# OzAmram/CaloDiffusion

Hardware: AMD Instinct MI355X
Metric: sampled showers/sec (Dataset-2, 400-step DDIM) (higher is better)
Workload: dtype f32 (convs: fp32 operands as 2-term fp16 splits on the fp16 MFMA pipe, fp32 accumulate; attention/norms fp32)

## Files before the change

### calodiffusion_amd/abi.py

```python
from __future__ import annotations

import ctypes as C
import os
from typing import Optional, Sequence

import torch

_HERE = os.path.dirname(os.path.abspath(__file__))
LIB_PATH = os.environ.get("CALODIFF_LIB") or os.path.join(_HERE, "lib", "libcalodiff_hip.so")

CD_MAX_SIZES = 8
CD_ABI_VERSION = 3
TIME_KINDS = {"log": 0, "sigma": 1, "raw": 2}
OBJECTIVES = {"hybrid": 0, "noise_pred": 1, "mean_pred": 2}
LOSS_TYPES = {"l2": 0, "l1": 1, "mse": 2, "huber": 3}


class CdUnetDesc(C.Structure):
    _fields_ = [
        ("struct_size", C.c_uint32),
        ("grid", C.c_int32 * 3),
        ("in_channels", C.c_int32),
        ("n_sizes", C.c_int32),
        ("layer_sizes", C.c_int32 * CD_MAX_SIZES),
# ... 22 lines not shown

class CdLayerMlpDesc(C.Structure):
    _fields_ = [("struct_size", C.c_uint32), ("dim_in", C.c_int32), ("hidden", C.c_int32), ("cond_emb", C.c_int32), ("cond_size", C.c_int32),
                ("n_res", C.c_int32), ("time_embed_kind", C.c_int32), ("objective", C.c_int32), ("sigma_data", C.c_float)]


class CdHlfDesc(C.Structure):
    _fields_ = [("struct_size", C.c_uint32), ("n_layers", C.c_int32), ("layer_offset", C.POINTER(C.c_int32)),
                ("eta", C.POINTER(C.c_double)), ("phi", C.POINTER(C.c_double)), ("with_centres", C.POINTER(C.c_int32))]


class CdGeneratorRun(C.Structure):
    _fields_ = [("struct_size", C.c_uint32), ("batch", C.c_int32), ("energy", C.c_void_p), ("energy_is_normalised", C.c_int32),
                ("sparse_mode", C.c_int32), ("layers", C.c_void_p), ("seed", C.c_uint64), ("offset", C.c_uint64),
                ("first_row", C.c_int32), ("global_batch", C.c_int32), ("showers", C.c_void_p), ("layers_out", C.c_void_p),
                ("next_offset", C.POINTER(C.c_uint64)), ("decode_seed", C.c_uint64), ("decode_offset", C.c_uint64),
                ("next_decode_offset", C.POINTER(C.c_uint64)), ("workspace", C.c_void_p), ("workspace_bytes", C.c_size_t),
                ("stream", C.c_void_p)]


class CdClassifierDesc(C.Structure):
    _fields_ = [("struct_size", C.c_uint32), ("input_dim", C.c_int32), ("hidden", C.c_int32), ("num_layer", C.c_int32),
                ("negative_slope", C.c_float), ("dropout_p", C.c_float)]


class CdStep(C.Structure):
    _fields_ = [("sigma", C.c_float), ("sigma_prev_masked", C.c_float), ("ddim_sigma", C.c_float), ("denom", C.c_float)]


_P = C.c_void_p
_SIGNATURES = {
    "cd_last_error": (C.c_char_p, []),
    "cd_abi_version": (C.c_int, []),
    "cd_device_check": (C.c_int, [C.c_char_p, C.c_int]),
    "cd_plan_create": (C.c_int, [C.POINTER(CdUnetDesc), C.POINTER(_P)]),
    "cd_plan_destroy": (C.c_int, [_P]),
    "cd_plan_num_weights": (C.c_int, [_P, C.POINTER(C.c_int)]),
    "cd_plan_weight_name": (C.c_int, [_P, C.c_int, C.c_char_p, C.c_int, C.POINTER(C.c_int64)]),
    "cd_plan_set_weight": (C.c_int, [_P, C.c_char_p, _P, C.c_int64, _P]),
    "cd_plan_set_weights": (C.c_int, [_P, C.c_int, C.POINTER(_P), _P]),
    "cd_plan_set_coords": (C.c_int, [_P, _P, _P, _P, _P]),
    "cd_plan_workspace_bytes": (C.c_int, [_P, C.c_int, C.POINTER(C.c_size_t)]),
    "cd_unet_forward": (C.c_int, [_P, C.c_int, _P, _P, _P, _P, _P, C.c_size_t, _P]),
    "cd_denoise": (C.c_int, [_P, C.c_int, _P, _P, _P, _P, _P, C.c_size_t, _P]),
    "cd_denoise_safe": (C.c_int, [_P, C.c_int, _P, _P, _P, _P, _P, C.c_size_t, C.POINTER(C.c_int), _P]),
    "cd_ddim_sample": (C.c_int, [_P, C.c_int, _P, _P, C.POINTER(CdStep), C.c_int, _P, C.c_uint64, C.c_uint64, C.c_uint64, _P, _P, _P,
                                 C.c_int, _P, C.c_size_t, _P]),
    "cd_plan_sampler_workspace_bytes": (C.c_int, [_P, C.c_int, C.c_int, C.c_int, C.c_int, C.POINTER(C.c_size_t)]),
    "cd_sampler_run": (C.c_int, [_P, C.c_int, _P, C.c_float, _P, C.c_int, C.c_int, C.POINTER(CdSamplerOp), C.c_int,
                                 C.POINTER(C.c_int32), _P, C.c_int, _P, C.c_uint64, C.c_uint64, C.c_uint64, _P, _P, _P, C.c_int,
                                 _P, C.c_size_t, _P]),
    "cd_randn": (C.c_int, [_P, C.c_int64, C.c_uint64, C.c_uint64, _P]),
    "cd_plan_grad_layout": (C.c_int, [_P, C.c_int, C.POINTER(C.c_int64), C.POINTER(C.c_int64)]),
    "cd_plan_train_workspace_bytes": (C.c_int, [_P, C.c_int, C.POINTER(C.c_size_t)]),
    "cd_plan_status": (C.c_int, [_P, C.POINTER(C.c_int), _P]),
    "cd_layer_forward": (C.c_int, [_P, C.POINTER(C.c_void_p), C.c_int, C.c_int, _P, _P, _P, _P, _P]),
    "cd_layer_denoise": (C.c_int, [_P, C.POINTER(C.c_void_p), C.c_int, C.c_int, _P, _P, _P, _P, _P]),
    "cd_layer_sample": (C.c_int, [_P, C.POINTER(C.c_void_p), C.c_int, C.c_int, _P, _P, _P, C.c_int, _P, _P, _P, _P, _P]),
    "cd_layer_sampler_run": (C.c_int, [_P, C.POINTER(C.c_void_p), C.c_int, C.c_int, _P, C.c_float, _P, C.c_int, C.c_int, _P, C.c_int,
                                       _P, _P, C.c_int, _P, C.c_uint64, C.c_uint64, C.c_uint64, _P, _P, _P, _P]),
    "cd_layer_train_workspace_bytes": (C.c_int, [_P, C.c_int, C.POINTER(C.c_size_t)]),
    "cd_layer_train_step": (C.c_int, [_P, C.POINTER(C.c_void_p), C.c_int, C.c_int, _P, _P, _P, _P, _P, _P, _P, C.c_size_t, _P]),
    "cd_layer_train_step_loss": (C.c_int, [_P, C.POINTER(C.c_void_p), C.c_int, C.c_int, _P, _P, _P, _P, C.c_int, _P, _P, _P, C.c_size_t,
                                           _P]),
    "cd_layer_loss": (C.c_int, [_P, C.POINTER(C.c_void_p), C.c_int, C.c_int, _P, _P, _P, _P, C.c_int, _P, _P, C.c_size_t, _P]),
    "cd_layer_vjp_workspace_bytes": (C.c_int, [_P, C.c_int, C.c_int, C.POINTER(C.c_size_t)]),
    "cd_layer_denoise_vjp": (C.c_int, [_P, C.POINTER(C.c_void_p), C.c_int, C.c_int, _P, _P, _P, _P, _P, _P, _P, C.c_size_t, _P]),
    "cd_reverse_norm": (C.c_int, [_P, _P, _P, _P, C.c_int, C.POINTER(C.c_int32), C.POINTER(C.c_float), C.c_float, C.c_float, _P]),
    "cd_reverse_norm_staged": (C.c_int, [_P, _P, _P, _P, C.c_int, C.POINTER(C.c_int32), C.POINTER(C.c_float), C.c_float, C.c_float,
                                         C.c_float, C.c_float, C.c_int, _P]),
    "cd_preprocess": (C.c_int, [_P, _P, _P, _P, _P, _P, C.c_int, C.POINTER(C.c_int32), C.POINTER(C.c_float), C.c_float, C.c_float,
                                C.c_float, C.c_int, C.c_float, _P]),
    "cd_preprocess_hgcal": (C.c_int, [_P, _P, C.c_int64, _P, C.c_int, _P, _P, _P, _P, C.c_int, C.c_int, C.c_int, C.c_int,
                                      C.POINTER(C.c_double), C.c_float, C.c_float, C.c_float, C.POINTER(C.c_double),
                                      C.POINTER(C.c_double), C.c_float, _P]),
    "cd_geom_create": (C.c_int, [_P, C.c_int, C.c_int, C.c_int, C.c_int, C.POINTER(_P), _P]),
    "cd_geom_create_ex": (C.c_int, [_P, _P, C.c_int, C.c_int, C.c_int, C.c_int, C.POINTER(_P), _P]),
    "cd_geom_create_csr": (C.c_int, [_P, _P, _P, C.c_int, C.c_int, C.c_int, C.c_int, C.POINTER(_P), _P]),
    "cd_geom_refresh": (C.c_int, [_P, _P, _P]),
    "cd_geom_destroy": (C.c_int, [_P]),
    "cd_geom_apply_vjp": (C.c_int, [_P, _P, _P, _P, _P, C.c_int, C.c_float, C.c_float, C.c_int, _P]),
    "cd_geom_apply": (C.c_int, [_P, _P, _P, C.c_int, C.c_float, C.c_float, C.c_int, _P]),
    "cd_geom_sparse_workspace_bytes": (C.c_int, [_P, C.c_int, C.POINTER(C.c_size_t)]),
    "cd_geom_decode_sparse": (C.c_int, [_P, _P, _P, C.c_int, C.c_int, C.c_int, _P, C.c_uint64, C.c_uint64, _P, _P]),
    "cd_radial_create": (C.c_int, [C.c_int, _P, _P, _P, C.c_int, C.c_int, C.POINTER(_P), _P]),
    "cd_radial_destroy": (C.c_int, [_P]),
    "cd_radial_enc": (C.c_int, [_P, _P, _P, _P, C.c_int, _P]),
    "cd_radial_dec": (C.c_int, [_P, _P, _P, _P, C.c_int, _P]),
    "cd_radial_enc_vjp": (C.c_int, [_P, _P, _P, _P, _P, _P, C.c_int, _P]),
    "cd_radial_dec_vjp": (C.c_int, [_P, _P, _P, _P, _P, _P, C.c_int, _P]),
    "cd_preprocess_ds1": (C.c_int, [_P, _P, _P, _P, _P, _P, _P, _P, C.c_int, C.POINTER(C.c_double), C.c_float, C.c_float, C.c_float,
                                    C.c_int, C.c_float, _P]),
    "cd_reverse_norm_ds1": (C.c_int, [_P, _P, _P, _P, _P, _P, C.c_int, C.POINTER(C.c_double), C.c_float, C.c_float, _P]),
    "cd_plan_set_radial": (C.c_int, [_P, _P, _P, _P, C.c_int, _P]),
    "cd_plan_set_geom": (C.c_int, [_P, _P, _P, C.c_int, _P]),
    "cd_adam_step": (C.c_int, [C.c_int, C.POINTER(C.c_void_p), C.POINTER(C.c_void_p), C.POINTER(C.c_void_p), C.POINTER(C.c_void_p),
                               C.POINTER(C.c_int64), C.c_double, C.c_double, C.c_double, C.c_float, C.c_float, C.c_int, _P]),
    "cd_train_step": (C.c_int, [_P, C.c_int, _P, _P, _P, _P, C.c_int, _P, _P, _P, C.c_size_t, _P]),
    "cd_plan_vjp_workspace_bytes": (C.c_int, [_P, C.c_int, C.c_int, C.POINTER(C.c_size_t)]),
    "cd_denoise_vjp": (C.c_int, [_P, C.c_int, _P, _P, _P, _P, _P, _P, _P, C.c_size_t, _P]),
    "cd_plan_bns_workspace_bytes": (C.c_int, [_P, C.c_int, C.c_int, C.POINTER(C.c_size_t)]),
    "cd_bns_theta_grad": (C.c_int, [_P, C.c_int, C.c_int, _P, _P, _P, _P, _P, _P, _P, C.c_size_t, _P]),
    "cd_generator_create": (C.c_int, [_P, C.c_size_t, C.POINTER(_P), _P]),
    "cd_generator_destroy": (C.c_int, [_P]),
    "cd_generator_checksum": (C.c_int, [_P, C.c_size_t, C.POINTER(C.c_uint64)]),
    "cd_generator_info": (C.c_int, [_P, C.POINTER(C.c_int32)]),
    "cd_generator_geometry": (C.c_int, [_P, C.POINTER(C.c_int32)]),
    "cd_generator_workspace_bytes": (C.c_int, [_P, C.c_int, C.POINTER(C.c_size_t)]),
    "cd_generator_run": (C.c_int, [_P, C.c_int, _P, C.c_int, _P, C.c_uint64, C.c_uint64, C.c_int, C.c_int, _P, _P, C.POINTER(C.c_uint64),
                                   _P, C.c_size_t, _P]),
    "cd_generator_run_ex": (C.c_int, [_P, C.POINTER(CdGeneratorRun)]),
    "cd_hlf_create": (C.c_int, [C.POINTER(CdHlfDesc), C.POINTER(_P), _P]),
    "cd_hlf_destroy": (C.c_int, [_P]),
    "cd_hlf_compute": (C.c_int, [_P, _P, C.c_int, C.c_float, _P, _P, _P]),
    "cd_fpd_workspace_bytes": (C.c_size_t, [C.c_int, C.c_int, C.c_int]),
    "cd_fpd_moments": (C.c_int, [_P, C.c_int64, C.c_int, _P, _P, C.c_int64, C.POINTER(C.c_int32), C.c_int, _P, _P, _P, _P, C.c_size_t, _P]),
    "cd_kpd_workspace_bytes": (C.c_size_t, [C.c_int, C.c_int]),
    "cd_kpd_sums": (C.c_int, [_P, C.c_int64, C.c_int, _P, C.c_int64, C.POINTER(C.c_int32), C.c_int, C.c_double, C.c_int, _P, _P, _P, C.c_size_t,
                              _P]),
    "cd_column_histograms_workspace_bytes": (C.c_size_t, [C.c_int64, C.c_int, C.c_int]),
    "cd_column_histograms": (C.c_int, [_P, C.c_int64, C.c_int64, C.c_int, _P, C.c_int, _P, _P, C.c_size_t, _P]),
    "cd_classifier_num_params": (C.c_int, [C.POINTER(CdClassifierDesc), C.POINTER(C.c_int64)]),
    "cd_classifier_workspace_bytes": (C.c_int, [C.POINTER(CdClassifierDesc), C.c_int, C.POINTER(C.c_size_t)]),
    "cd_classifier_forward": (C.c_int, [C.POINTER(CdClassifierDesc), C.POINTER(C.c_void_p), _P, C.c_int64, _P, C.c_int64, _P, C.c_int, _P,
                                        C.c_size_t, _P]),
    "cd_classifier_train_step": (C.c_int, [C.POINTER(CdClassifierDesc), C.POINTER(C.c_void_p), _P, _P, C.c_int64, _P, C.c_int, C.c_uint64,
                                           C.c_uint64, _P, _P, C.c_int, _P, _P, C.c_double, C.c_double, C.c_double, C.c_float, C.c_int, _P,
                                           C.c_size_t, _P]),
    "cd_classifier_train_epoch": (C.c_int, [C.POINTER(CdClassifierDesc), C.POINTER(C.c_void_p), _P, _P, C.c_int64, _P, C.c_int64, C.c_int,
                                            C.c_uint64, C.c_uint64, _P, _P, _P, C.c_double, C.c_double, C.c_double, C.c_float, _P, _P,
                                            C.c_size_t, _P]),
    "cd_classifier_dropout_mask": (C.c_int, [C.c_uint64, C.c_uint64, C.c_int, C.c_float, C.c_int, C.c_int, _P, _P]),
    "cd_set_conv_precision": (C.c_int, [C.c_char_p]),
    "cd_get_conv_precision": (C.c_char_p, []),
    "cd_profile_begin": (C.c_int, []),
    "cd_profile_end": (C.c_int, [C.c_char_p, C.c_int]),
    "cd_loss_hybrid_l2": (C.c_int, [_P, C.c_int, _P, _P, _P, _P, _P, _P, C.c_size_t, _P]),
    "cd_loss_hybrid": (C.c_int, [_P, C.c_int, _P, _P, _P, _P, C.c_int, _P, _P, C.c_size_t, _P]),
    "cd_op_to_channels_last": (C.c_int, [_P, _P, C.c_int, C.c_int, C.c_int64, _P]),
    "cd_op_to_ncdhw": (C.c_int, [_P, _P, C.c_int, C.c_int, C.c_int64, _P]),
    "cd_op_cyl_conv": (C.c_int, [_P, C.c_int, _P, C.c_int, _P, _P, _P, C.c_int, C.c_int, C.POINTER(C.c_int32),
                                 C.POINTER(C.c_int32), C.POINTER(C.c_int32), _P, _P]),
    "cd_op_zslide_conv": (C.c_int, [_P, C.c_int, _P, _P, _P, _P, C.POINTER(C.c_int), C.c_int, C.c_int, C.POINTER(C.c_int32), C.c_int,
                                    _P, _P]),
    "cd_op_cyl_conv_transpose": (C.c_int, [_P, _P, _P, _P, C.c_int, C.c_int, C.POINTER(C.c_int32), C.c_int, C.c_int,
                                           C.POINTER(C.c_int32), _P, _P]),
    "cd_op_init_conv": (C.c_int, [_P, _P, _P, _P, C.c_int, C.c_int, C.c_int, C.POINTER(C.c_int32), _P, _P]),
    "cd_op_init_pair_conv": (C.c_int, [_P, _P, _P, _P, _P, C.c_int, _P, _P, _P, C.c_int, C.c_int, _P, _P, _P, C.POINTER(C.c_int), C.c_int,
                                       C.POINTER(C.c_int32), C.c_int, _P, _P]),
    "cd_op_group_norm": (C.c_int, [_P, _P, _P, _P, C.c_int, C.c_int, C.c_int64, C.c_int, C.c_int, _P, _P, _P, _P]),
    "cd_op_resnet_block": (C.c_int, [_P, C.c_int, _P, C.c_int, C.POINTER(_P), _P, _P, C.c_int, C.c_int,
                                     C.POINTER(C.c_int32), C.c_int, _P, C.c_size_t, _P]),
    "cd_op_linear_attention": (C.c_int, [_P, C.POINTER(_P), _P, C.c_int, C.c_int, C.POINTER(C.c_int32), _P, C.c_size_t, _P]),
    "cd_op_conv_backward": (C.c_int, [_P, C.c_int, _P, C.c_int, _P, _P, _P, _P, _P, C.c_int, C.c_int, C.POINTER(C.c_int32),
                                      C.POINTER(C.c_int32), C.POINTER(C.c_int32), _P, C.c_size_t, _P]),
    "cd_op_conv_transpose_backward": (C.c_int, [_P, _P, _P, _P, _P, _P, C.c_int, C.c_int, C.POINTER(C.c_int32), C.c_int, C.c_int,
                                                C.POINTER(C.c_int32), _P, C.c_size_t, _P]),
    "cd_op_group_norm_backward": (C.c_int, [_P, _P, _P, _P, _P, _P, _P, _P, C.c_int, C.c_int, C.c_int64, C.c_int, C.c_int, _P,
                                            C.c_size_t, _P]),
    "cd_op_scratch_bytes": (C.c_size_t, [C.c_int, C.c_int, C.c_int64]),
    "cd_op_linear_act": (C.c_int, [_P, _P, _P, _P, C.c_int, C.c_int, C.c_int, C.c_int, C.c_float, C.c_float, C.c_uint64, C.c_uint64, C.c_int,
                                   _P]),
    "cd_op_linear_act_backward": (C.c_int, [_P, _P, _P, _P, _P, C.c_float, C.c_int, C.c_float, _P, _P, _P, C.c_int, C.c_int, C.c_int, _P,
                                            C.c_size_t, _P]),
}
EXPORTED_SYMBOLS = tuple(_SIGNATURES)

_lib = None


def load_library() -> C.CDLL:
    global _lib
    if _lib is not None:
        return _lib
    if not os.path.exists(LIB_PATH):
        raise RuntimeError(
            f"{LIB_PATH} is missing: build it with `python -m calodiffusion_amd.build` (hipcc, --offload-arch=gfx950). "
            "calodiffusion_amd has no CPU or PyTorch fallback.")
    _check_built_from_these_sources()
    lib = C.CDLL(LIB_PATH)
    for name, (res, args) in _SIGNATURES.items():
        fn = getattr(lib, name)
        fn.restype, fn.argtypes = res, args
    if lib.cd_abi_version() != CD_ABI_VERSION:
        raise RuntimeError(f"{LIB_PATH} reports ABI version {lib.cd_abi_version()}, this binding is written against "
                           f"{CD_ABI_VERSION} (include/calodiff.h): rebuild with `python -m calodiffusion_amd.build`")
    _lib = lib
    return lib


def _check_built_from_these_sources():
    if os.environ.get("CALODIFF_LIB") or os.environ.get("CD_SKIP_SRCHASH"):
        return
    from . import build
    stamp = LIB_PATH + ".srchash"
    have = open(stamp).read().strip() if os.path.exists(stamp) else None
    want = build.source_hash()
    if have != want:
        raise RuntimeError(f"{LIB_PATH} was not built from the sources in {build.CSRC} (stamp {str(have)[:12]}, sources "
                           f"{want[:12]}): run `python -m calodiffusion_amd.build`")


def _check(code: int):
    if code != 0:
        msg = load_library().cd_last_error().decode(errors="replace")
        exc = ValueError if code == -1 else RuntimeError
        raise exc(f"calodiff[{code}]: {msg}")


def require_gpu() -> str:
    lib = load_library()
    if not torch.cuda.is_available():
        raise RuntimeError("calodiffusion_amd needs an MI355X (gfx950) GPU: torch.cuda.is_available() is False and "
                           "there is no CPU fallback")
    buf = C.create_string_buffer(256)
    _check(lib.cd_device_check(buf, 256))
    return buf.value.decode()


def _ptr(t: Optional[torch.Tensor]) -> Optional[int]:
    return None if t is None else t.data_ptr()


def _stream() -> int:
    return torch.cuda.current_stream().cuda_stream


def _dev32(t: torch.Tensor, name: str) -> torch.Tensor:
    if not isinstance(t, torch.Tensor) or not t.is_cuda:
        raise RuntimeError(f"{name} must be a CUDA(ROCm) tensor: calodiffusion_amd computes on the GPU only")
    if t.dtype != torch.float32 or not t.is_contiguous():
        t = t.to(torch.float32).contiguous()
    return t


def _i32x3(v: Sequence[int]):
    return (C.c_int32 * 3)(*[int(a) for a in v])


class WorkspaceCache:

    def __init__(self):
        self._kept = {}

    def get(self, kind, key, device, nbytes) -> torch.Tensor:
        key = tuple(key)
        kept = self._kept.get(kind)
        if kept is not None and kept[0] == key and (callable(nbytes) or kept[1].numel() >= nbytes):
            return kept[1]
        del kept
        self._kept.pop(kind, None)
        ws = torch.empty(int(nbytes() if callable(nbytes) else nbytes), dtype=torch.uint8, device=device)
        self._kept[kind] = (key, ws)
        return ws

    def drop(self, *kinds):
        for kind in kinds:
            self._kept.pop(kind, None)

    def clear(self):
        self._kept.clear()

    def __iter__(self):
        return iter([(kind,) + key for kind, (key, _) in self._kept.items()])

    def __len__(self):
        return len(self._kept)


def set_conv_precision(mode: str):
    _check(load_library().cd_set_conv_precision(mode.encode()))


def get_conv_precision() -> str:
    return load_library().cd_get_conv_precision().decode()


def profile_begin():
    _check(load_library().cd_profile_begin())


def profile_end() -> dict:
    import json
    buf = C.create_string_buffer(1 << 18)
    _check(load_library().cd_profile_end(buf, 1 << 18))
    return json.loads(buf.value.decode())


def randn(shape, device, seed: int, offset: int = 0) -> torch.Tensor:
    lib = load_library()
    require_gpu()
    out = torch.empty(tuple(shape), dtype=torch.float32, device=device)
    _check(lib.cd_randn(out.data_ptr(), out.numel(), int(seed), int(offset), _stream()))
    return out
```

### calodiffusion_amd/csrc/forward.hip

```cpp
#include "plan_internal.h"
#include "kernels_attn.h"
#include "kernels_deep.h"
#include "kernels_loss.h"

#include <cstdio>
#include <cstdlib>

namespace cd {

ResP resolve(const CdPlan* p, const ResW& w, const float* emb) {
  ResP r;
  r.cin = w.cin; r.cout = w.cout; r.has_res = w.has_res;
  r.c1w3 = p->packed3(w.c1w); r.c2w3 = p->packed3(w.c2w);
  r.c1w = p->packed(w.c1w); r.c1b = p->raw(w.c1b); r.n1g = p->raw(w.n1g); r.n1b = p->raw(w.n1b);
  r.c2w = p->packed(w.c2w); r.c2b = p->raw(w.c2b); r.n2g = p->raw(w.n2g); r.n2b = p->raw(w.n2b);
  if (w.has_res) {
    r.rw = p->packed(w.rw); r.rb = p->raw(w.rb);
    if (p->packed3(w.rw)) r.rw16 = (const char*)p->packed3(w.rw) + packed_bf16x3_bytes(w.cin, w.cout, 1);
  }
  if (w.has_mlp && emb) { r.emb = emb + w.emb_off; r.emb_ld = p->emb_ld; }
  return r;
}
AttnP resolve(const CdPlan* p, const AttnW& w) {
  AttnP a;
  a.c = w.c;
  a.ng = p->raw(w.ng); a.nb = p->raw(w.nb); a.qkv = p->packed(w.qkv); a.ow = p->raw(w.ow); a.ob = p->raw(w.ob);
  a.qkv16 = (const char*)p->packed3(w.qkv) + packed_bf16x3_bytes(w.c, 96, 1);
  a.gg = p->raw(w.gg); a.gb = p->raw(w.gb);
  a.coop_sync = p->d_attn_sync;
  return a;
}

float* stats_pass(Run& r, const float* x, int C, int64_t vox, int* units) {
  const int ns = gn_nsplit_for(vox, r.B);
  float* part = r.ws->get<float>((size_t)r.B * ns * C * 2);
  if (!r.dry()) launch_ch_stats(x, part, r.B, C, vox, ns, r.s);
  *units = ns;
  return part;
}

float* conv3_with_stats(Run& r, const float* x0, int c0, const float* x1, int c1, const float* wpk, const void* wpk3,
                        const float* bias, float* out, int cout, Dims3 dims, const float* coef_in, int* units,
                        const GnDefer* defer_in, float* coef_buf, const ConvFusion::GnOut* gn_out) {
  const int64_t vox = dims.vox();
  const int cap = (int)((vox + 31) / 32);
  float* part = r.ws->get<float>((size_t)r.B * cap * cout * 2);
  int u = 0;
  if (!r.dry()) {
    ConvGeom g{dims, dims, 3, 3, 3, 1, 1, 1};
    ConvFusion fu;
    fu.coef = coef_in; fu.act = 1; fu.ch_part = part; fu.units = &u; fu.wpk_bf16x3 = wpk3; fu.status = r.status;
    if (defer_in) { fu.defer = *defer_in; fu.coef_buf = coef_buf; fu.coef = nullptr; }
    if (gn_out) fu.gn_out = *gn_out;
    launch_conv_mfma(x0, c0, x1, c1, wpk, bias, out, r.B, cout, g, r.s, fu);
    if (gn_out && *gn_out->done) {
    } else if (u == 0) {
      u = gn_nsplit_for(vox, r.B);
      if (u > cap) u = cap;
      launch_ch_stats(out, part, r.B, cout, vox, u, r.s);
    }
  }
  *units = u;
  return part;
}

static float* conv3_x_half_with_stats(Run& r, const float* x0, int c0, int c1, const void* wpk3, float* out, int cout, Dims3 dims,
                                      int* units) {
  const int64_t vox = dims.vox();
  const int cap = (int)((vox + 31) / 32);
  float* part = r.ws->get<float>((size_t)r.B * cap * cout * 2);
  int u = 0;
  if (!r.dry()) {
    ConvGeom g{dims, dims, 3, 3, 3, 1, 1, 1};
    ConvFusion fu;
    int added = 0;
    fu.act = 1; fu.ch_part = part; fu.units = &u; fu.status = r.status; fu.add_src = out; fu.add_done = &added;
    char cat[128];
    std::snprintf(cat, sizeof cat, "conv3x3x3_s1 C%d(of %d)->%d @%dx%dx%d", c0, c0 + c1, cout, dims.d, dims.h, dims.w);
    prof::Scope scope(cat, r.s, 2.0 * 27 * c0 * cout * (double)vox * r.B, 4.0 * r.B * (double)vox * (c0 + 2 * cout));
    const bool ran = try_launch_conv_zslide(x0, c0, nullptr, 0, (const char*)wpk3 + packed_bf16x3_bytes(c0 + c1, cout, 27), nullptr, out,
                                            r.B, cout, g, r.s, fu);
    CD_REQUIRE(ran && added && u > 0, "internal: the x half of a side conv must run as a z-slide continuation");
  }
  *units = u;
  return part;
}

struct LazyClose {
  GnDefer gn;
  float* part = nullptr;
  bool on = false;
};
float* res_block(Run& r, const ResP& w, const float* x0, int c0, const float* x1, int c1, Dims3 dims,
                 float** part_out, int* units_out, LazyClose* lazy, float* h1_side, const ConvDone* h1_done) {
  Arena* ws = r.ws;
  CD_REQUIRE(c0 + c1 == w.cin, "internal: resnet block input width mismatch");
  const int64_t vox = dims.vox();
  const int G = r.groups;
  int u1 = 0, u2 = 0;
  static const bool defer_gn = getenv("CD_NO_GNDEFER") == nullptr;
  float* h1 = h1_done ? h1_done->h1 : (h1_side ? h1_side : ws->get<float>((size_t)r.B * vox * w.cout));
  const bool whole = vox <= 128 && w.cout == 32 && defer_gn && conv_precision() == PREC_F16X2 && w.c1w3 && w.c2w3;
  float* p1 = nullptr;
  CD_REQUIRE(!h1_side || (!whole && c1 > 0), "internal: a side conv belongs to a concat conv on a full-resolution grid");
  CD_REQUIRE(!h1_done || (!whole && !h1_side && c1 == 0), "internal: a finished first conv belongs to a single-input block on a full-resolution grid");
  if (h1_done) { p1 = h1_done->part; u1 = h1_done->units; }
  else if (h1_side) p1 = conv3_x_half_with_stats(r, x0, c0, c1, w.c1w3, h1, w.cout, dims, &u1);
  else if (!whole) p1 = conv3_with_stats(r, x0, c0, x1, c1, w.c1w, w.c1w3, w.c1b, h1, w.cout, dims, nullptr, &u1);
  else p1 = ws->get<float>((size_t)r.B * ((vox + 31) / 32) * w.cout * 2);
  float* coef1 = ws->get<float>((size_t)r.B * w.cout * 4);
  GnDefer d1;
  d1.part = p1; d1.units = u1; d1.gamma = w.n1g; d1.beta = w.n1b; d1.add = w.emb; d1.add_ld = w.emb_ld; d1.C = w.cout; d1.groups = G;
  d1.vox = vox;
  if (!r.dry() && !defer_gn) launch_gn_finalize(p1, u1, w.n1g, w.n1b, w.emb, w.emb_ld, coef1, r.B, w.cout, G, vox, r.s);
  float* h2 = ws->get<float>((size_t)r.B * vox * w.cout);
  const bool small = vox <= 128;
  float* po = nullptr;
  const bool no_pw_close = getenv("CD_NO_PW_CLOSE") != nullptr;
  const bool pw_close = w.has_res && !small && defer_gn && !no_pw_close && w.cout <= 128;
  const int bps = pw_close ? pointwise_units(vox) : gn_apply_blocks_per_sample(r.B, w.cout, vox);
  if (part_out) {
    po = ws->get<float>((size_t)r.B * bps * w.cout * 2);
    *part_out = po;
  }
  float* res = nullptr;
  auto shortcut_conv = [&](const GnDefer* close = nullptr) {
    if (!close) res = ws->get<float>((size_t)r.B * vox * w.cout);
    if (!r.dry()) {
      PointwiseArgs a;
      a.in0 = x0; a.ld0 = c0; a.off0 = 0; a.c0 = c0; a.in1 = x1; a.ld1 = c1; a.c1 = c1;
      a.wpk = w.rw; a.bias = w.rb; a.out = close ? h2 : res; a.batch = r.B; a.cout = w.cout; a.vox = vox;
      if (conv_precision() == PREC_F16X2 && !getenv("CD_PW_F32")) { a.wpk16 = w.rw16; a.status = r.status; }
      if (close) { a.gn_res = h2; a.gn_defer = *close; a.ch_part = po; }
      launch_pointwise(a, r.s);
    }
  };
  if (small && w.has_res) shortcut_conv();
  int fused = 0;
  if (whole && !r.dry()) {
    const float* sc0 = w.has_res ? res : x0;
    const float* sc1 = w.has_res ? nullptr : (c1 ? x1 : nullptr);
    if (try_launch_res_block_small(x0, c0, x1, c1, (const char*)w.c1w3 + packed_bf16x3_bytes(c0 + c1, 32, 27), w.c1b, w.n1g, w.n1b,
                                   w.emb, w.emb_ld, (const char*)w.c2w3 + packed_bf16x3_bytes(32, 32, 27), w.c2b, w.n2g, w.n2b, G, sc0,
                                   sc1, w.has_res ? 0 : c0, h1, h2, po, r.B, w.cout, dims, r.status, r.s))
      fused = 2;
    else
      p1 = (ws->release(p1), conv3_with_stats(r, x0, c0, x1, c1, w.c1w, w.c1w3, w.c1b, h1, w.cout, dims, nullptr, &u1));
  }
  ConvFusion::GnOut go;
  if (small && defer_gn && fused != 2) {
    go.gamma = w.n2g; go.beta = w.n2b; go.groups = G; go.part_out = po; go.done = &fused;
    if (w.has_res) { go.res0 = res; }
    else { go.res0 = x0; go.res1 = c1 ? x1 : nullptr; go.res_c0 = c0; }
  }
  float* p2 = nullptr;
  if (fused == 2) p2 = ws->get<float>((size_t)r.B * ((vox + 31) / 32) * w.cout * 2);
  else p2 = conv3_with_stats(r, h1, w.cout, nullptr, 0, w.c2w, w.c2w3, w.c2b, h2, w.cout, dims, coef1, &u2, defer_gn ? &d1 : nullptr,
                             coef1, go.gamma ? &go : nullptr);
  ws->release(p1);
  ws->release(h1);
  ws->release(coef1);
  float* coef2 = ws->get<float>((size_t)r.B * w.cout * 4);
  GnDefer d2;
  d2.part = p2; d2.units = u2; d2.gamma = w.n2g; d2.beta = w.n2b; d2.C = w.cout; d2.groups = G; d2.vox = vox;
  if (!r.dry() && !defer_gn) launch_gn_finalize(p2, u2, w.n2g, w.n2b, nullptr, 0, coef2, r.B, w.cout, G, vox, r.s);
  const GnDefer* dp2 = defer_gn ? &d2 : nullptr;
  if (part_out) *units_out = fused ? 1 : bps;
  if (pw_close) {
    shortcut_conv(&d2);
  } else if (w.has_res) {
    if (!res) shortcut_conv();
    if (!r.dry() && !fused) launch_gn_apply(h2, h2, coef2, r.B, w.cout, vox, 1, res, nullptr, 0, po, r.s, dp2);
    ws->release(res);
  } else if (lazy && !small && defer_gn && c1 == 0 && w.cout == 32 && !part_out) {
    lazy->gn = d2;
    lazy->part = p2;
    lazy->on = true;
    ws->release(coef2);
    return h2;
  } else {
    if (!r.dry() && !fused) launch_gn_apply(h2, h2, coef2, r.B, w.cout, vox, 1, x0, c1 ? x1 : nullptr, c0, po, r.s, dp2);
  }
  ws->release(p2);
  ws->release(coef2);
  return h2;
}

float* attn_block(Run& r, const AttnP& w, const float* x, Dims3 dims, float* xpart, int xunits) {
  Arena* ws = r.ws;
  const int64_t vox = dims.vox();
  const int C = w.c;
  float* own = nullptr;
  if (!xpart) {
    own = stats_pass(r, x, C, vox, &xunits);
    xpart = own;
  }
  static const bool no_fused_env = getenv("CD_NO_FUSED_ATTN") != nullptr;
  static const bool defer_env = getenv("CD_NO_GNDEFER") == nullptr;
  const bool no_fused = no_fused_env || conv_precision() != PREC_F16X2;
  const bool defer_gn = defer_env && !no_fused;
  float* coefn = ws->get<float>((size_t)r.B * C * 4);
  GnDefer dn;
  dn.part = xpart; dn.units = xunits; dn.gamma = w.ng; dn.beta = w.nb; dn.C = C; dn.groups = 1; dn.vox = vox;
  const GnDefer* dnp = defer_gn ? &dn : nullptr;
  if (!r.dry() && !defer_gn) launch_gn_finalize(xpart, xunits, w.ng, w.nb, nullptr, 0, coefn, r.B, C, 1, vox, r.s);
  const int CT = (C + 31) / 32;
  float* y = nullptr;
  float* ypart = nullptr;
  int yu = 0;
  const bool single = !no_fused && defer_gn && attn_small_eligible(vox);
  bool moments = false;
  if (!no_fused) {
    const int nsp = attn_fused_nsplit_for(vox, r.B);
    const int cap = single && nsp < 4 ? 4 : nsp;
    float* part = ws->get<float>(attn_partial_floats(r.B, cap));
    static const bool sep_combine = getenv("CD_ATTN_COMBINE_LAUNCH") != nullptr;
    const char* mom_env = getenv("CD_ATTN_MOM_MIN");
    const int64_t mom_min = mom_env ? atoll(mom_env) : (4ll << 20);
    moments = !single && !sep_combine && defer_gn && attn_moments_eligible(C) && (vox * C) % 4 == 0 && (int64_t)r.B * vox * C >= mom_min &&
              getenv("CD_NO_ATTN_MOMENTS") == nullptr;
    float* momb = moments ? ws->get<float>(attn_moment_floats(r.B, nsp)) : nullptr;
    float* wpb = ws->get<float>((size_t)r.B * CT * 1024);
    y = ws->get<float>((size_t)r.B * vox * C);
    yu = nsp;
    ypart = ws->get<float>((size_t)r.B * cap * C * 2);
    if (!r.dry() && single) {
      launch_attn_small(x, C, coefn, w.qkv16, part, w.ow, kAttnScale, w.ob, w.gg, w.gb, y, ypart, r.B, vox,
                        r.s, dnp, r.status, cap, w.coop_sync);
    } else if (!r.dry()) {
      launch_attn_kv_context(x, C, coefn, w.qkv16, part, r.B, vox, nsp, r.s, dnp, r.status, momb);
      if (sep_combine) {
        launch_attn_combine(part, nsp, w.ow, C, wpb, r.B, kAttnScale, r.s, nullptr, nullptr, true);
        launch_attn_out(x, C, coefn, w.qkv16, wpb, w.ob, y, ypart, r.B, vox, nsp, r.s, dnp, nullptr, nullptr, 0.f, r.status);
      } else {
        launch_attn_out(x, C, coefn, w.qkv16, nullptr, w.ob, y, moments ? nullptr : ypart, r.B, vox, nsp, r.s, dnp, part, w.ow,
                        kAttnScale, r.status, momb, w.gg, w.gb);
      }
    }
    if (momb) ws->release(momb);
    if (own) ws->release(own);
    own = nullptr;
    ws->release(coefn);
    ws->release(part);
    ws->release(wpb);
  } else {
    float* qkv = ws->get<float>((size_t)r.B * vox * 96);
    ws->release(coefn);
    const int nsp = attn_nsplit_for(vox, r.B);
    float* part = ws->get<float>(attn_partial_floats(r.B, nsp));
    float* wpb = ws->get<float>((size_t)r.B * CT * 1024);
    y = ws->get<float>((size_t)r.B * vox * C);
    yu = pointwise_units(vox);
    ypart = ws->get<float>((size_t)r.B * yu * C * 2);
    if (!r.dry()) launch_attn_unfused(x, C, coefn, w.qkv, w.ow, w.ob, qkv, part, nsp, wpb, y, ypart, r.B, vox, r.s);
    ws->release(part);
    ws->release(wpb);
    ws->release(qkv);
}
  if (own) ws->release(own);
  float* coefg = ws->get<float>((size_t)r.B * C * 4);
  if (!r.dry() && !single && !moments) {
    GnDefer dg;
    dg.part = ypart; dg.units = yu; dg.gamma = w.gg; dg.beta = w.gb; dg.C = C; dg.groups = 1; dg.vox = vox;
    if (!defer_gn) launch_gn_finalize(ypart, yu, w.gg, w.gb, nullptr, 0, coefg, r.B, C, 1, vox, r.s);
    launch_gn_apply(y, y, coefg, r.B, C, vox, 0, x, nullptr, 0, nullptr, r.s, defer_gn ? &dg : nullptr);
  }
  ws->release(ypart);
  ws->release(coefg);
  return y;
}

bool deep_level_desc(const CdPlan* p, const float* emb, DeepLevelDesc* out) {
  const CdUnetDesc& d = p->desc;
  const int nres = p->nres;
  if (conv_precision() != PREC_F16X2) return false;
  DeepLevelDesc L;
  L.dims = p->shapes[nres - 1];
  L.Ca = d.layer_sizes[nres - 1]; L.Cb = d.layer_sizes[nres]; L.groups = d.groups;
  const ResW* rw[6] = {&p->downs[nres - 1].r1, &p->downs[nres - 1].r2, &p->mid1, &p->mid2, &p->ups[0].r1, &p->ups[0].r2};
  for (int i = 0; i < 6; ++i) {
    const ResW& w = *rw[i];
    DeepLevelDesc::Res& r = L.res[i];
    const bool cat = i == 4;
    r.c0 = cat ? L.Cb : w.cin; r.c1 = cat ? w.cin - L.Cb : 0; r.cout = w.cout;
    if (!p->packed3(w.c1w) || !p->packed3(w.c2w)) return false;
    r.w1 = (const char*)p->packed3(w.c1w) + packed_bf16x3_bytes(w.cin, w.cout, 27);
    r.w2 = (const char*)p->packed3(w.c2w) + packed_bf16x3_bytes(w.cout, w.cout, 27);
    r.b1 = p->raw(w.c1b); r.b2 = p->raw(w.c2b); r.g1 = p->raw(w.n1g); r.be1 = p->raw(w.n1b); r.g2 = p->raw(w.n2g); r.be2 = p->raw(w.n2b);
    if (w.has_mlp && emb) { r.emb = emb + w.emb_off; r.emb_ld = p->emb_ld; }
    if (w.has_res) {
      if (!p->packed3(w.rw)) return false;
      r.wres = (const char*)p->packed3(w.rw) + packed_bf16x3_bytes(w.cin, w.cout, 1);
      r.bres = p->raw(w.rb);
    }
  }
  const AttnW* aw[3] = {&p->downs[nres - 1].attn, &p->mid_attn, &p->ups[0].attn};
  const bool on[3] = {d.block_attn != 0, d.mid_attn != 0, d.block_attn != 0};
  for (int i = 0; i < 3; ++i) {
    L.has_attn[i] = on[i] ? 1 : 0;
    if (!on[i]) continue;
    const AttnW& w = *aw[i];
    DeepLevelDesc::Attn& a = L.attn[i];
    a.C = w.c; a.ng = p->raw(w.ng); a.nb = p->raw(w.nb); a.wout = p->raw(w.ow); a.bout = p->raw(w.ob); a.gg = p->raw(w.gg); a.gb = p->raw(w.gb);
    if (!p->packed3(w.qkv)) return false;
    a.wqkv = (const char*)p->packed3(w.qkv) + packed_bf16x3_bytes(w.c, 96, 1);
  }
  if (L.res[0].c0 != L.Ca || L.res[0].cout != L.Cb || L.res[4].cout != L.Ca || L.res[4].c1 != L.Cb || L.res[5].cout != L.Ca) return false;
  if (!deep_level_eligible(L)) return false;
  *out = L;
  return true;
}

float* unet_body(CdPlan* p, Run& r, const float* emb, float* h, LazyClose* lazy = nullptr, float** xin = nullptr,
                 const ConvDone* first = nullptr) {
  const CdUnetDesc& d = p->desc;
  const int nres = p->nres;
  const int zs = d.compress_z ? 2 : 1;
  std::vector<float*> skips(nres, nullptr);
  float* x = h;
  int cx = d.layer_sizes[0];
  DeepLevelDesc deep;
  const bool deep_on = deep_level_desc(p, emb, &deep);
  const ResW& side_w = p->ups[nres - 1].r1;
  const int side_c = nres >= 2 ? d.layer_sizes[1] : 0;
  const bool side_on = deep_on && nres >= 2 && side_w.cin == 2 * side_c && p->packed3(side_w.c1w) &&
                       deep_side_conv_chunks(r.B, side_c, side_w.cout, p->shapes[0]) > 0;
  float* side_h1 = nullptr;
  for (int i = 0; i < nres; ++i) {
    const Dims3 dims = p->shapes[i];
    if (deep_on && i == nres - 1) {
      float* y = r.ws->get<float>((size_t)r.B * dims.vox() * cx);
      if (side_on) {
        side_h1 = r.ws->get<float>((size_t)r.B * p->shapes[0].vox() * side_w.cout);
        if (!r.dry()) {
          DeepSideConv sc;
          sc.in = skips[0]; sc.ldc = side_c; sc.cin = side_c;
          sc.wpk = (const char*)p->packed3(side_w.c1w) + packed_bf16x3_bytes(side_w.cin, side_w.cout, 27) +
                   (size_t)(side_c / 16) * 27 * (side_w.cout / 32) * 128 * 16;
          sc.bias = p->raw(side_w.c1b); sc.out = side_h1; sc.cout = side_w.cout; sc.dims = p->shapes[0];
          launch_deep_level_side(deep, x, y, r.B, r.status, sc, r.s);
        }
      } else if (!r.dry()) {
        launch_deep_level(deep, x, y, r.B, r.status, r.s);
      }
      r.ws->release(x);
      x = y;
      break;
    }
    float* t = res_block(r, resolve(p, p->downs[i].r1, emb), x, cx, nullptr, 0, dims, nullptr, nullptr, nullptr, nullptr,
                         i == 0 ? first : nullptr);
    r.ws->release(x);
    x = t; cx = p->downs[i].r1.cout;
    float* xp = nullptr;
    int xu = 0;
    t = res_block(r, resolve(p, p->downs[i].r2, emb), x, cx, nullptr, 0, dims, d.block_attn ? &xp : nullptr, &xu);
    r.ws->release(x);
    x = t;
    if (d.block_attn) {
      t = attn_block(r, resolve(p, p->downs[i].attn), x, dims, xp, xu);
      r.ws->release(xp);
      r.ws->release(x);
      x = t;
    }
    skips[i] = x;
    if (i + 1 < nres) {
      const Dims3 nd = p->shapes[i + 1];
      float* y = r.ws->get<float>((size_t)r.B * nd.vox() * cx);
      if (!r.dry()) {
        ConvGeom g{dims, nd, 3, 4, 4, zs, 2, 2};
        ConvFusion fu;
        fu.wpk_bf16x3 = p->packed3(p->downs[i].sw);
        launch_conv_mfma(x, cx, nullptr, 0, p->packed(p->downs[i].sw), p->raw(p->downs[i].sb), y, r.B, cx, g, r.s, fu);
      }
      x = y;
    } else {
      x = skips[i];
    }
  }
  const Dims3 md = p->shapes[nres - 1];
  float* t = nullptr;
  if (!deep_on) {
    float* mp = nullptr;
    int mu = 0;
    t = res_block(r, resolve(p, p->mid1, emb), x, cx, nullptr, 0, md, d.mid_attn ? &mp : nullptr, &mu);
    x = t;
    if (d.mid_attn) {
      t = attn_block(r, resolve(p, p->mid_attn), x, md, mp, mu);
      r.ws->release(mp);
      r.ws->release(x);
      x = t;
    }
    t = res_block(r, resolve(p, p->mid2, emb), x, cx, nullptr, 0, md);
    r.ws->release(x);
    x = t;
  }

  for (int i = 0; i < nres; ++i) {
    const int lv = nres - 1 - i;
    const Dims3 dims = p->shapes[lv];
    const int cs = d.layer_sizes[lv + 1];
    if (!(deep_on && i == 0)) {
      CD_REQUIRE(cx == cs, "internal: up path width mismatch");
      t = res_block(r, resolve(p, p->ups[i].r1, emb), x, cx, skips[lv], cs, dims, nullptr, nullptr, nullptr,
                    lv == 0 ? side_h1 : nullptr);
      r.ws->release(x);
      r.ws->release(skips[lv]);
      x = t; cx = p->ups[i].r1.cout;
      float* up = nullptr;
      int uu = 0;
      t = res_block(r, resolve(p, p->ups[i].r2, emb), x, cx, nullptr, 0, dims, d.block_attn ? &up : nullptr, &uu);
      r.ws->release(x);
      x = t;
      if (d.block_attn) {
        t = attn_block(r, resolve(p, p->ups[i].attn), x, dims, up, uu);
        r.ws->release(up);
        r.ws->release(x);
        x = t;
      }
    }
    if (i + 1 < nres) {
      const Dims3 od = p->up_out[i];
      float* y = r.ws->get<float>((size_t)r.B * od.vox() * cx);
      if (!r.dry())
        launch_conv_transpose_mfma(x, cx, p->packed(p->ups[i].sw), p->raw(p->ups[i].sb), y, r.B, cx, dims, od, p->up_kz[i], zs, r.s,
                                   p->packed3(p->ups[i].sw), r.status);
      r.ws->release(x);
      x = y;
    }
  }
  t = res_block(r, resolve(p, p->fin, nullptr), x, cx, nullptr, 0, p->shapes[0], nullptr, nullptr, lazy);
  if (lazy && lazy->on) *xin = x;
  else r.ws->release(x);
  return t;
}

EmbedArgs embed_args(CdPlan* p, int B, const float* cond, const float* t, int kind, float* emb, float* scal) {
  const CdUnetDesc& d = p->desc;
  EmbedArgs e;
  e.cond = cond; e.time_or_sigma = t; e.time_kind = kind; e.sigma_data = d.sigma_data;
  e.cond_size = d.cond_size; e.half = d.cond_dim / 2;
  e.cond_hidden = d.cond_size > e.half / 2 ? d.cond_size : e.half / 2;
  e.time_sin = d.time_sin; e.cond_sin = d.cond_sin;
  e.tw1 = d.time_sin ? nullptr : p->raw(p->tw[0]); e.tb1 = d.time_sin ? nullptr : p->raw(p->tb[0]);
  e.tw2 = p->raw(p->tw[1]); e.tb2 = p->raw(p->tb[1]);
  e.tw3 = p->raw(p->tw[2]); e.tb3 = p->raw(p->tb[2]);
  e.cw1 = d.cond_sin ? nullptr : p->raw(p->cw[0]); e.cb1 = d.cond_sin ? nullptr : p->raw(p->cb[0]);
  e.cw2 = p->raw(p->cw[1]); e.cb2 = p->raw(p->cb[1]);
  e.cw3 = p->raw(p->cw[2]); e.cb3 = p->raw(p->cb[2]);
  e.layers = p->d_embed_layers; e.n_layers = p->n_embed_layers; e.emb = emb; e.emb_ld = p->emb_ld; e.scal = scal; e.batch = B;
  return e;
}

void forward_impl(CdPlan* p, int B, const float* x, const float* cond, const float* t, float* out, bool raw, hipStream_t s,
                  const FwdOpts* opt) {
  const CdUnetDesc& d = p->desc;
  const Dims3 dims = p->shapes[0];
  Run r{&p->ws, s, B, d.groups};
  r.status = p->status_word;
  const bool pre = opt && opt->emb_pre;
  float* emb = pre ? opt->emb_pre : p->ws.get<float>((size_t)B * p->emb_ld);
  float* scal = pre ? opt->scal_pre : p->ws.get<float>((size_t)B * 4);
  float* h = p->ws.get<float>((size_t)B * dims.vox() * d.layer_sizes[0]);
  const CdPlan::FlatEmbed* fe = raw ? nullptr : p->flat();
  float* g_in = fe ? p->ws.get<float>((size_t)B * dims.vox()) : nullptr;
  float* f_grid = fe ? p->ws.get<float>((size_t)B * dims.vox()) : nullptr;
  if (!r.dry()) {
    if (!pre) launch_embed(embed_args(p, B, cond, t, raw ? CD_TIME_RAW : d.time_embed_kind, emb, raw ? nullptr : scal), s);
    if (fe) launch_embed_in(*fe, x, scal, g_in, B, s);
    InitConvArgs a;
    a.x = fe ? g_in : x; a.cin = d.in_channels; a.wpk = p->packed(p->init_w); a.bias = p->raw(p->init_b); a.out = h; a.batch = B;
    a.cout = d.layer_sizes[0]; a.dims = dims;
    if (raw) {
      a.cx = d.in_channels;
    } else {
      a.cx = 1; a.sigma_b = fe ? nullptr : t; a.sigma_data = d.sigma_data; a.use_rz = d.rz_input; a.use_phi = d.phi_input;
      a.r_w = p->d_coords; a.z_d = p->d_coords + d.grid[2]; a.phi_h = p->d_coords + d.grid[2] + d.grid[0];
      a.coord_table = p->d_init_table; a.table_ready = true; a.status = r.status;
    }
    launch_init_conv(a, s);
  }
  ConvDone pair;
  const bool pair_on = !raw && p->d_pair_w && p->init_pair_ready && conv_precision() == PREC_F16X2 && getenv("CD_NO_INIT_PAIR") == nullptr;
  if (pair_on) {
    pair.h1 = p->ws.get<float>((size_t)B * dims.vox() * 32);
    pair.part = p->ws.get<float>((size_t)B * ((dims.vox() + 31) / 32) * 32 * 2);
    if (!r.dry()) {
      InitPairArgs ia;
      ia.x = fe ? g_in : x; ia.sigma_b = fe ? nullptr : t; ia.sigma_data = d.sigma_data;
      ia.wc = p->d_pair_w; ia.table = p->d_pair_table; ia.out = pair.h1; ia.ch_part = pair.part; ia.batch = B; ia.dims = dims;
      ia.status = r.status;
      launch_init_pair_conv(ia, &pair.units, s);
    }
  }
  LazyClose lazy;
  float* xin = nullptr;
  static const bool head_fused = getenv("CD_NO_HEAD_GN") == nullptr;
  float* hf = unet_body(p, r, emb, h, head_fused ? &lazy : nullptr, &xin, pair_on ? &pair : nullptr);
  if (!r.dry()) {
    HeadArgs ha;
    ha.h = hf; ha.w = p->raw(p->head_w); ha.bias = p->raw(p->head_b); ha.out = fe ? f_grid : out; ha.batch = B; ha.vox = dims.vox();
    if (!raw && !fe) { ha.x = x; ha.scal = scal; ha.objective = d.objective; }
    if (lazy.on) { ha.defer = lazy.gn; ha.res = xin; }
    if (opt && opt->upd && !fe) {
      ha.upd_stepvals = opt->upd->upd_stepvals; ha.upd_noise = opt->upd->upd_noise; ha.upd_x_next = opt->upd->upd_x_next;
      ha.upd_xs = opt->upd->upd_xs; ha.upd_x0s = opt->upd->upd_x0s;
    }
    launch_head(ha, s);
    if (fe) launch_embed_out(*fe, f_grid, x, scal, d.objective, out, opt ? opt->upd : nullptr, B, s);
  }
  if (fe) {
    r.ws->release(f_grid);
    r.ws->release(g_in);
  }
  if (lazy.on) {
    r.ws->release(lazy.part);
    r.ws->release(xin);
  }
  r.ws->release(hf);
  if (!pre) {
    r.ws->release(scal);
    r.ws->release(emb);
  }
}

}

extern "C" {

int cd_plan_workspace_bytes(CdPlan* plan, int batch, size_t* bytes) {
  return guarded([&] {
    CD_REQUIRE(plan && bytes && batch > 0, "bad argument");
    const int64_t n = (int64_t)batch * plan->state_per();
    *bytes = dry_forward_bytes(plan, batch, [&] {
      plan->ws.get<float>((size_t)n);
      plan->ws.get<float>((size_t)n);
      plan->ws.get<float>((size_t)batch + 64);
      plan->ws.get<double>((size_t)batch + 8);
      plan->ws.get<float>((size_t)batch * plan->emb_ld);
      plan->ws.get<float>((size_t)batch * 4);
      plan->ws.get<float>((size_t)CdPlan::kEmbedChunk * batch * plan->emb_ld);
      plan->ws.get<float>((size_t)CdPlan::kEmbedChunk * batch * 4);
    }) + 4096;
  });
}

int cd_unet_forward(CdPlan* plan, int batch, const float* x, const float* cond, const float* time, float* out,
                    void* workspace, size_t workspace_bytes, void* stream) {
  return guarded([&] {
    CD_REQUIRE(plan && x && cond && time && out && workspace && batch > 0, "bad argument");
    check_ready(plan, false);
    plan->ws.reset((char*)workspace, workspace_bytes, false);
    forward_impl(plan, batch, x, cond, time, out, true, (hipStream_t)stream);
  });
}

int cd_denoise(CdPlan* plan, int batch, const float* x, const float* sigma, const float* cond, float* out,
               void* workspace, size_t workspace_bytes, void* stream) {
  return guarded([&] {
    CD_REQUIRE(plan && x && sigma && cond && out && workspace && batch > 0, "bad argument");
    check_ready(plan, true);
    plan->ws.reset((char*)workspace, workspace_bytes, false);
    forward_impl(plan, batch, x, cond, sigma, out, false, (hipStream_t)stream);
  });
}

int cd_denoise_safe(CdPlan* plan, int batch, const float* x, const float* sigma, const float* cond, float* out,
                    void* workspace, size_t workspace_bytes, int* fell_back, void* stream) {
  return guarded([&] {
// ... 39 lines not shown
```

### calodiffusion_amd/csrc/kernels_attn.h

```cpp
#pragma once
#include "cd_common.h"
#include "kernels_gn.h"

namespace cd {

constexpr float kAttnScale = 0.17677669529663689f;

int attn_nsplit_for(int64_t vox, int batch);
size_t attn_partial_floats(int batch, int nsplit);
void launch_attn_context(const float* qkv, float* partials, int batch, int64_t vox, int nsplit, hipStream_t s);
void launch_attn_combine(const float* partials, int nsplit, const float* w_out , int cout, float* wpk_b,
                         int batch, float scale, hipStream_t s, float* ctx_out = nullptr ,
                         float* kstat_out = nullptr ,
                         bool layout_T = false );
void launch_attn_unfused(const float* x, int C, const float* coef, const float* wqkv, const float* w_out, const float* bias,
                         float* qkv, float* partials, int nsplit, float* wpk_b, float* y, float* ch_part, int batch, int64_t vox,
                         hipStream_t s, float* ctx_out = nullptr, float* kstat_out = nullptr);

int attn_fused_nsplit_for(int64_t vox, int batch);
bool attn_small_eligible(int64_t vox);
void launch_attn_small(const float* x, int C, const float* coef, const void* wqkv_f16x2, float* partials, const float* w_out,
                       float scale, const float* bias, const float* out_gamma, const float* out_beta, float* y, float* ch_part,
                       int batch, int64_t vox, hipStream_t s, const GnDefer* defer, int* status = nullptr,
                       int max_parts = 1, unsigned* coop_sync = nullptr);
constexpr int kAttnCoopSamples = 8192;
bool attn_moments_eligible(int C);
size_t attn_moment_floats(int batch, int nsplit);
void launch_attn_kv_context(const float* x, int C, const float* coef, const void* wqkv_f16x2, float* partials, int batch,
                            int64_t vox, int nsplit, hipStream_t s, const GnDefer* defer = nullptr, int* status = nullptr,
                            float* moments = nullptr);
void launch_attn_out(const float* x, int C, const float* coef, const void* wqkv_f16x2, const float* wT_b, const float* bias,
                     float* y, float* ch_part , int batch, int64_t vox, int nsplit, hipStream_t s,
                     const GnDefer* defer = nullptr,
                     const float* partials = nullptr, const float* w_out = nullptr, float scale = 0.f, int* status = nullptr,
                     const float* moments = nullptr, const float* out_gamma = nullptr, const float* out_beta = nullptr);

}
```

### calodiffusion_amd/csrc/kernels_attn.hip

```cpp
#include "kernels_attn.h"
#include "gn_defer.h"
#include "split16.h"

#include <cstdio>
#include <cstdlib>

namespace cd {

namespace {

struct AttnArgs {
  const float* x;
  const float* coef;
  const u32x4* wqkv;
  int C;
  int64_t vox;
  int tiles_per_wg;
  float* partials;
  int nsplit;
  const float* wT;
  const float* fold_wout;
  float fold_scale;
  const float* bias;
  float* y;
  float* ch_part;
  GnDefer defer;
  const float *out_gamma, *out_beta;
  int* status;
  unsigned* sync;
  int coop;
  float* mom;
};
constexpr int ATTN_MOM = 32 + 1024;
__device__ __forceinline__ float attn_peer_load(const float* p, int coop) {
  return coop ? __hip_atomic_load(p, __ATOMIC_RELAXED, __HIP_MEMORY_SCOPE_AGENT) : *p;
}

template <int NCH>
struct RawTile {
  f32x4 v[NCH * 2][2];
};
template <int NCH>
__device__ __forceinline__ void load_raw(const AttnArgs& a, int b, int64_t t, int64_t tlast, int col, int half, RawTile<NCH>& raw) {
  const int64_t tc = t < tlast ? t : tlast;
  int64_t n = tc * 32 + col;
  n = n < a.vox ? n : a.vox - 1;
  const float* src = a.x + ((size_t)b * a.vox + n) * a.C + half * 8;
#pragma unroll
  for (int ks = 0; ks < NCH * 2; ++ks)
#pragma unroll
    for (int j = 0; j < 2; ++j) raw.v[ks][j] = *(const f32x4*)(src + ks * 16 + j * 4);
}
template <int NCH, bool CFL = false>
__device__ __forceinline__ void norm_split(const AttnArgs& a, int64_t n0, int col, const f32x4 (&cf)[NCH][8], const RawTile<NCH>& raw,
                                           u32x4 (&x1)[NCH * 2], u32x4 (&x2)[NCH * 2], float& amax, const f32x4* cf_lds = nullptr) {
  const bool valid = n0 + col < a.vox;
#pragma unroll
  for (int ks = 0; ks < NCH * 2; ++ks) {
    u32x2 t1[2], t2[2];
#pragma unroll
    for (int j = 0; j < 2; ++j) {
      f32x4 v = raw.v[ks][j];
#pragma unroll
      for (int e = 0; e < 4; ++e) {
        const f32x4 c2 = CFL ? cf_lds[(ks >> 1) * 8 + (ks & 1) * 4 + j * 2 + (e >> 1)] : cf[ks >> 1][(ks & 1) * 4 + j * 2 + (e >> 1)];
        v[e] = valid ? c2[(e & 1) * 2] * v[e] + c2[(e & 1) * 2 + 1] : 0.f;
      }
      amax = fmaxf(amax, fmaxf(fmaxf(fabsf(v[0]), fabsf(v[1])), fmaxf(fabsf(v[2]), fabsf(v[3]))));
      split2(v, t1[j], t2[j]);
    }
    x1[ks] = u32x4{t1[0][0], t1[0][1], t1[1][0], t1[1][1]};
    x2[ks] = u32x4{t2[0][0], t2[0][1], t2[1][0], t2[1][1]};
  }
}
#ifndef ATTN_OUT_D1
#define ATTN_OUT_D1 0
#endif
template <int NCH>
struct AttnDepthOut {
  static constexpr int value = NCH == 1 ? ATTN_OUT_D1 : 0;
};
__device__ __forceinline__ float attn_exp(float x) {
  const float L2E = 1.4426950408889634f, L2E_LO = 1.925963033500519e-8f;
  const float t = x * L2E;
  const float lo = __builtin_fmaf(x, L2E, -t) + x * L2E_LO;
  const float e = __builtin_amdgcn_exp2f(t);
  return __builtin_fmaf(e, lo * 0.6931471805599453f, e);
}
__device__ __forceinline__ void attn_barrier_lds() { asm volatile("s_waitcnt lgkmcnt(0)\n\ts_barrier" ::: "memory"); }
template <int NCH>
__device__ __forceinline__ void load_coef(const AttnArgs& a, int b, int half, f32x4 (&cf)[NCH][8]) {
  __shared__ __attribute__((aligned(16))) float sCoef[NCH * 32 * 4];
  __shared__ __attribute__((aligned(16))) char sDefer[NCH * 32 * 16 + 64 * 8];
  const float* base = a.defer.part ? nullptr : a.coef + (size_t)b * a.C * 4;
  if (a.defer.part) {
    gn_defer_to_lds(a.defer, b, sCoef, sDefer);
    base = sCoef;
  }
#pragma unroll
  for (int ch = 0; ch < NCH; ++ch)
#pragma unroll
    for (int i = 0; i < 8; ++i) {
      const float* p = base + (ch * 32 + (i >> 2) * 16 + half * 8 + 2 * (i & 3)) * 4;
      cf[ch][i] = f32x4{p[0], p[1], p[4], p[5]};
    }
}

template <int NCH, bool MOM>
struct AttnCfl {
  static constexpr bool value = MOM || NCH >= 2;
};
template <int NCH>
__device__ __forceinline__ const f32x4* attn_cf_table(const f32x4 (&cf)[NCH][8], f32x4* table) {
  const int lane = threadIdx.x & 63, half = lane >> 5;
  if (threadIdx.x < 64 && (lane & 31) == 0) {
#pragma unroll
    for (int ch = 0; ch < NCH; ++ch)
#pragma unroll
      for (int i = 0; i < 8; ++i) table[(half * NCH + ch) * 8 + i] = cf[ch][i];
  }
  __syncthreads();
  return table + half * NCH * 8;
}

template <int NCH, bool MOM = false>
__device__ __forceinline__ void attn_pass1(const AttnArgs& a, int b, int split, int64_t t0, int64_t t1, const f32x4 (&cf)[NCH][8],
                                           const f32x4* cf_lds = nullptr ) {
  __shared__ float sMax[8][32];
  __shared__ float sSum[16][32];
  __shared__ float sCtx[8][1024];
  const int tid = threadIdx.x, lane = tid & 63, wave = __builtin_amdgcn_readfirstlane(tid >> 6);
  const int half = lane >> 5, col = lane & 31;
  constexpr int NKS = NCH * 2;
  u32x4 wk1[NKS], wk2[NKS], wv1[NKS], wv2[NKS];
#pragma unroll
  for (int ks = 0; ks < NKS; ++ks) {
    wk1[ks] = a.wqkv[(size_t)(ks * 3 + 1) * 128 + lane];
    wk2[ks] = a.wqkv[(size_t)(ks * 3 + 1) * 128 + 64 + lane];
    wv1[ks] = a.wqkv[(size_t)(ks * 3 + 2) * 128 + lane];
    wv2[ks] = a.wqkv[(size_t)(ks * 3 + 2) * 128 + 64 + lane];
  }
  u32x4 wq1[MOM ? NKS : 1], wq2[MOM ? NKS : 1];
  __shared__ __attribute__((aligned(16))) float sQt[MOM ? 8 * 32 * 36 : 4];
  f32x16 mS, mSB;
  float msum = 0.f;
  if constexpr (MOM) {
#pragma unroll
    for (int ks = 0; ks < NKS; ++ks) {
      wq1[ks] = a.wqkv[(size_t)(ks * 3 + 0) * 128 + lane];
      wq2[ks] = a.wqkv[(size_t)(ks * 3 + 0) * 128 + 64 + lane];
    }
#pragma unroll
    for (int r = 0; r < 16; ++r) mS[r] = mSB[r] = 0.f;
  }
  const f32x16 zero16 = {0.f, 0.f, 0.f, 0.f, 0.f, 0.f, 0.f, 0.f, 0.f, 0.f, 0.f, 0.f, 0.f, 0.f, 0.f, 0.f};
  auto project = [&](const u32x4 (&x1)[NKS], const u32x4 (&x2)[NKS], const u32x4 (&w1)[NKS], const u32x4 (&w2)[NKS]) {
    f32x16 pa = zero16, pb = zero16;
#pragma unroll
    for (int ks = 0; ks < NKS; ++ks) {
      pa = MFMA_F16(x1[ks], w1[ks], pa);
      pb = MFMA_F16(x1[ks], w2[ks], pb);
      pb = MFMA_F16(x2[ks], w1[ks], pb);
    }
#pragma unroll
    for (int r = 0; r < 16; ++r) pa[r] += pb[r] * (1.f / 2048.f);
    return pa;
  };

  __shared__ __attribute__((aligned(16))) float sFac[8][32];
  RawTile<NCH> raw;
  const int64_t tlast = t1 - 1;
  float m = -3.0e38f;
  bool any = false;
  float amax = 0.f;
  f32x16 ctx, ctxB;
#pragma unroll
  for (int r = 0; r < 16; ++r) ctx[r] = ctxB[r] = 0.f;
  float ssum = 0.f;
  auto scale_rows = [&](float fac) {
    sFac[wave][col] = fac;
    asm volatile("s_waitcnt lgkmcnt(0)" ::: "memory");
#pragma unroll
    for (int q = 0; q < 4; ++q) {
      const f32x4 f4 = *(const f32x4*)&sFac[wave][8 * q + 4 * half];
#pragma unroll
      for (int e = 0; e < 4; ++e) {
        ctx[4 * q + e] *= f4[e];
        ctxB[4 * q + e] *= f4[e];
      }
    }
  };
  auto split8 = [](const float (&x)[16], int s8, u32x4& hi, u32x4& lo) {
    u32x2 h0, l0, h1, l1;
    split2(f32x4{x[8 * s8], x[8 * s8 + 1], x[8 * s8 + 2], x[8 * s8 + 3]}, h0, l0);
    split2(f32x4{x[8 * s8 + 4], x[8 * s8 + 5], x[8 * s8 + 6], x[8 * s8 + 7]}, h1, l1);
    hi = u32x4{h0[0], h0[1], h1[0], h1[1]};
    lo = u32x4{l0[0], l0[1], l1[0], l1[1]};
  };
  for (int64_t tt = t0 + wave; tt < t1; tt += 8) {
    u32x4 x1[NKS], x2[NKS];
    load_raw<NCH>(a, b, tt, tlast, col, half, raw);
    norm_split<NCH, AttnCfl<NCH, MOM>::value>(a, tt * 32, col, cf, raw, x1, x2, amax, cf_lds);
    const f32x16 k = project(x1, x2, wk1, wk2);
    const f32x16 v = project(x1, x2, wv1, wv2);
    const bool full = tt * 32 + 32 <= a.vox;
    float tm = -3.0e38f;
#pragma unroll
    for (int r = 0; r < 16; ++r) {
      const int row = (r & 3) + 8 * (r >> 2) + 4 * half;
      if (full || tt * 32 + row < a.vox) tm = fmaxf(tm, k[r]);
    }
    tm = fmaxf(tm, __shfl_xor(tm, 32, 64));
    if (!any) {
      m = tm;
      any = true;
    } else if (__builtin_amdgcn_ballot_w64(tm > m) != 0) {
      const float mn = fmaxf(m, tm);
      const float fac = attn_exp(m - mn);
      ssum *= fac;
      scale_rows(fac);
      m = mn;
    }
    float ex[16], vv[16];
#pragma unroll
    for (int r = 0; r < 16; ++r) {
      const int row = (r & 3) + 8 * (r >> 2) + 4 * half;
      ex[r] = (full || tt * 32 + row < a.vox) ? attn_exp(k[r] - m) : 0.f;
      ssum += ex[r];
      vv[r] = v[r];
      amax = fmaxf(amax, fabsf(v[r]));
    }
#pragma unroll
    for (int s8 = 0; s8 < 2; ++s8) {
      u32x4 e1, e2, v1, v2;
      split8(ex, s8, e1, e2);
      split8(vv, s8, v1, v2);
      ctx = MFMA_F16(e1, v1, ctx);
      ctxB = MFMA_F16(e1, v2, ctxB);
      ctxB = MFMA_F16(e2, v1, ctxB);
    }
    if constexpr (MOM) {
      f32x16 q = zero16, qb = zero16;
#pragma unroll
      for (int ks = 0; ks < NKS; ++ks) {
        q = MFMA_F16(wq1[ks], x1[ks], q);
        qb = MFMA_F16(wq2[ks], x1[ks], qb);
        qb = MFMA_F16(wq1[ks], x2[ks], qb);
      }
#pragma unroll
      for (int r = 0; r < 16; ++r) q[r] += qb[r] * (1.f / 2048.f);
      float mx = q[0];
#pragma unroll
      for (int r = 1; r < 16; ++r) mx = fmaxf(mx, q[r]);
      mx = fmaxf(mx, __shfl_xor(mx, 32, 64));
      float ss = 0.f;
#pragma unroll
      for (int r = 0; r < 16; ++r) {
        q[r] = __builtin_amdgcn_exp2f((q[r] - mx) * 1.4426950408889634f);
// ... 254 lines not shown
  for (int ct = 0; ct < NCH; ++ct) {
    bv[ct] = a.bias ? a.bias[ct * 32 + col] : 0.f;
    s1[ct] = s2[ct] = 0.f;
    osc[ct] = 1.f;
    if constexpr (MOM) {
      osc[ct] = sOut[ct * 32 + col][0];
      bv[ct] = sOut[ct * 32 + col][1];
    }
  }
  float* const yb = a.y + (size_t)b * a.vox * a.C;
  const float* const xb = a.x + (size_t)b * a.vox * a.C;

  constexpr int PRE = AttnDepthOut<NCH>::value, DEPTH = PRE ? PRE : 1;
  RawTile<NCH> raw[DEPTH];
  const int64_t tlast = t1 - 1;
  if (PRE) {
#pragma unroll
    for (int d = 0; d < DEPTH; ++d) load_raw<NCH>(a, b, t0 + wave + 8 * d, tlast, col, half, raw[d]);
  }
  for (int64_t tg = t0 + wave; tg < t1; tg += 8 * DEPTH) {
#pragma unroll
  for (int d = 0; d < DEPTH; ++d) {
    const int64_t t = tg + 8 * d;
    if (t >= t1) break;
    u32x4 x1[NKS], x2[NKS];
    if (!PRE) load_raw<NCH>(a, b, t, tlast, col, half, raw[d]);
    norm_split<NCH, AttnCfl<NCH, MOM>::value>(a, t * 32, col, cf, raw[d], x1, x2, amax, cf_lds);
    if (PRE && t + 8 * DEPTH < t1) load_raw<NCH>(a, b, t + 8 * DEPTH, tlast, col, half, raw[d]);
    f32x16 q = zero16, qb = zero16;
#pragma unroll
    for (int ks = 0; ks < NKS; ++ks) {
      q = MFMA_F16(wq1[ks], x1[ks], q);
      qb = MFMA_F16(wq2[ks], x1[ks], qb);
      qb = MFMA_F16(wq1[ks], x2[ks], qb);
    }
#pragma unroll
    for (int r = 0; r < 16; ++r) q[r] += qb[r] * (1.f / 2048.f);
    float mx = q[0];
#pragma unroll
    for (int r = 1; r < 16; ++r) mx = fmaxf(mx, q[r]);
    mx = fmaxf(mx, __shfl_xor(mx, 32, 64));
    float ss = 0.f;
#pragma unroll
    for (int r = 0; r < 16; ++r) {
      q[r] = attn_exp(q[r] - mx);
      ss += q[r];
    }
    ss += __shfl_xor(ss, 32, 64);
    const float inv = 1.f / ss;
    u32x4 p1[2], p2[2];
#pragma unroll
    for (int s8 = 0; s8 < 2; ++s8) {
      u32x2 h0, l0, h1, l1;
      split2(f32x4{q[8 * s8] * inv, q[8 * s8 + 1] * inv, q[8 * s8 + 2] * inv, q[8 * s8 + 3] * inv}, h0, l0);
      split2(f32x4{q[8 * s8 + 4] * inv, q[8 * s8 + 5] * inv, q[8 * s8 + 6] * inv, q[8 * s8 + 7] * inv}, h1, l1);
      p1[s8] = u32x4{h0[0], h0[1], h1[0], h1[1]};
      p2[s8] = u32x4{l0[0], l0[1], l1[0], l1[1]};
    }
#pragma unroll
    for (int ct = 0; ct < NCH; ++ct) {
      f32x16 o = zero16, ob = zero16;
#pragma unroll
      for (int s8 = 0; s8 < 2; ++s8) {
        o = MFMA_F16(p1[s8], wb1[ct][s8], o);
        ob = MFMA_F16(p1[s8], wb2[ct][s8], ob);
        ob = MFMA_F16(p2[s8], wb1[ct][s8], ob);
      }
#pragma unroll
      for (int r = 0; r < 16; ++r) o[r] += ob[r] * (1.f / 2048.f);
      if (trbuf && t * 32 + 32 <= a.vox) {
        float* tr = trbuf + wave * (32 * 36);
        const size_t qoff = (size_t)t * 32 * a.C + ct * 32 + (lane & 7) * 4;
        f32x4 xres[4];
        if constexpr (MOM) {
#pragma unroll
          for (int k = 0; k < 4; ++k) xres[k] = *(const f32x4*)(xb + qoff + (size_t)(8 * k + (lane >> 3)) * a.C);
        }
#pragma unroll
        for (int r = 0; r < 16; ++r) {
          const float v = MOM ? __builtin_fmaf(o[r], osc[ct], bv[ct]) : o[r] + bv[ct];
          tr[((r & 3) + 8 * (r >> 2) + 4 * half) * 36 + col] = v;
          if (!MOM) {
            s1[ct] += v;
            s2[ct] += v * v;
          }
        }
        asm volatile("s_waitcnt lgkmcnt(0)" ::: "memory");
        float* yt = yb + qoff;
#pragma unroll
        for (int k = 0; k < 4; ++k) {
          const int row = 8 * k + (lane >> 3);
          f32x4 v4 = *(const f32x4*)(tr + row * 36 + (lane & 7) * 4);
          if constexpr (MOM) v4 += xres[k];
          *(f32x4*)(yt + (size_t)row * a.C) = v4;
        }
        asm volatile("s_waitcnt lgkmcnt(0)" ::: "memory");
      } else {
#pragma unroll
      for (int r = 0; r < 16; ++r) {
        const int64_t n = t * 32 + (r & 3) + 8 * (r >> 2) + 4 * half;
        if (n < a.vox) {
          const size_t at = (size_t)n * a.C + ct * 32 + col;
          const float v = MOM ? __builtin_fmaf(o[r], osc[ct], bv[ct]) + xb[at] : o[r] + bv[ct];
          yb[at] = v;
          s1[ct] += v;
          s2[ct] += v * v;
        }
      }
      }
    }
  }
  }
  if (a.status && !(amax <= 65504.f)) atomicOr(a.status, 1);
  if constexpr (!MOM) if (a.ch_part) {
#pragma unroll
    for (int ct = 0; ct < NCH; ++ct) {
      const float t1s = s1[ct] + __shfl_xor(s1[ct], 32, 64), t2s = s2[ct] + __shfl_xor(s2[ct], 32, 64);
      if (half == 0) {
        sRed[wave][ct * 32 + col][0] = t1s;
        sRed[wave][ct * 32 + col][1] = t2s;
      }
    }
    __syncthreads();
    if (tid < NCH * 32) {
      float r1 = 0.f, r2 = 0.f;
#pragma unroll
      for (int w = 0; w < 8; ++w) {
        r1 += sRed[w][tid][0];
        r2 += sRed[w][tid][1];
      }
      float* dst = a.ch_part + (((size_t)b * nunits + unit) * a.C + tid) * 2;
      dst[0] = r1;
      dst[1] = r2;
    }
  }
}

template <int NCH, bool MOM>
__global__ void __launch_bounds__(512) attn_out_kernel(AttnArgs a) {
  const int half = (threadIdx.x & 63) >> 5;
  const int unit = blockIdx.x, b = blockIdx.y;
  const int64_t T = (a.vox + 31) / 32;
  const int64_t t0 = (int64_t)unit * a.tiles_per_wg;
  const int64_t t1 = (t0 + a.tiles_per_wg < T) ? t0 + a.tiles_per_wg : T;
  f32x4 cf[NCH][8];
  load_coef<NCH>(a, b, half, cf);
  __shared__ __attribute__((aligned(16))) float sTr[8 * 32 * 36];
  __shared__ __attribute__((aligned(16))) f32x4 sCfT[2 * NCH * 8];
  const f32x4* cfl = nullptr;
  if constexpr (AttnCfl<NCH, MOM>::value) cfl = attn_cf_table<NCH>(cf, sCfT);
  attn_pass2<NCH, MOM>(a, b, unit, (int)gridDim.x, t0, t1, cf, sTr, cfl);
}

template <int NCH>
__global__ void __launch_bounds__(512) attn_small_kernel(AttnArgs a) {
  __shared__ __attribute__((aligned(16))) float sOut[NCH * 32][2];
  __shared__ double sTot[2];
  const int tid = threadIdx.x, half = (tid & 63) >> 5;
  const int b = blockIdx.x;
  const int64_t T = (a.vox + 31) / 32;
  f32x4 cf[NCH][8];
  load_coef<NCH>(a, b, half, cf);
  __shared__ __attribute__((aligned(16))) f32x4 sCfT[2 * NCH * 8];
  const f32x4* cfl = nullptr;
  if constexpr (AttnCfl<NCH, false>::value) cfl = attn_cf_table<NCH>(cf, sCfT);
  attn_pass1<NCH>(a, b, 0, 0, T, cf, cfl);
  __threadfence_block();
  __syncthreads();
  attn_pass2<NCH>(a, b, 0, 1, 0, T, cf, nullptr, cfl);
  __threadfence_block();
  __syncthreads();
  const int C = NCH * 32;
  const float* cp = a.ch_part + (size_t)b * C * 2;
  if (tid < 64) {
    double a1 = 0.0, a2 = 0.0;
    for (int c = tid; c < C; c += 64) {
      const float2 v = *(const float2*)(cp + c * 2);
      a1 += (double)v.x;
      a2 += (double)v.y;
    }
#pragma unroll
    for (int m = 32; m >= 1; m >>= 1) {
      a1 += __shfl_xor(a1, m, 64);
      a2 += __shfl_xor(a2, m, 64);
    }
    if (tid == 0) {
      const double cnt = (double)a.vox * C;
      const double mu = a1 / cnt;
      double var = a2 / cnt - mu * mu;
      var = var < 0.0 ? 0.0 : var;
      sTot[0] = mu;
      sTot[1] = 1.0 / sqrt(var + 1e-5);
    }
  }
  __syncthreads();
  if (tid < C) {
    const float sc = (float)sTot[1] * a.out_gamma[tid];
    sOut[tid][0] = sc;
    sOut[tid][1] = a.out_beta[tid] - (float)sTot[0] * sc;
  }
  __syncthreads();
  float* const yb = a.y + (size_t)b * a.vox * C;
  const float* const xb = a.x + (size_t)b * a.vox * C;
  const int64_t n4 = a.vox * C / 4;
  for (int64_t i = tid; i < n4; i += 512) {
    const int c = (int)((i * 4) % C);
    const f32x4 y = ((const f32x4*)yb)[i], x = ((const f32x4*)xb)[i];
    f32x4 o;
#pragma unroll
    for (int e = 0; e < 4; ++e) o[e] = sOut[c + e][0] * y[e] + sOut[c + e][1] + x[e];
    ((f32x4*)yb)[i] = o;
  }
}

__device__ __forceinline__ void attn_group_barrier(unsigned* sync, int P, int* status) {
  asm volatile("s_waitcnt vmcnt(0)" ::: "memory");
  __syncthreads();
  if (threadIdx.x == 0) {
    const unsigned g = __hip_atomic_load(sync + 1, __ATOMIC_RELAXED, __HIP_MEMORY_SCOPE_AGENT);
    const unsigned arrived = __hip_atomic_fetch_add(sync, 1u, __ATOMIC_RELAXED, __HIP_MEMORY_SCOPE_AGENT);
    if (arrived == (unsigned)P - 1) {
      __hip_atomic_store(sync, 0u, __ATOMIC_RELAXED, __HIP_MEMORY_SCOPE_AGENT);
      asm volatile("s_waitcnt vmcnt(0)" ::: "memory");
      __hip_atomic_fetch_add(sync + 1, 1u, __ATOMIC_RELAXED, __HIP_MEMORY_SCOPE_AGENT);
    } else {
      int spins = 0;
      while (__hip_atomic_load(sync + 1, __ATOMIC_RELAXED, __HIP_MEMORY_SCOPE_AGENT) == g) {
        __builtin_amdgcn_s_sleep(1);
        if (++spins > (1 << 21)) {
          if (status) atomicOr(status, 1);
          break;
        }
      }
    }
  }
  __syncthreads();
}

template <int NCH>
__global__ void __launch_bounds__(512) attn_coop_kernel(AttnArgs a) {
  __shared__ __attribute__((aligned(16))) float sOut[NCH * 32][2];
  __shared__ double sTot[2];
  const int tid = threadIdx.x, half = (tid & 63) >> 5;
  const int P = a.nsplit;
  const int xcd = blockIdx.x & 7, slot = blockIdx.x >> 3;
  const int b = (slot / P) * 8 + xcd, part = slot % P;
  const int64_t T = (a.vox + 31) / 32;
  const int64_t t0 = (int64_t)part * a.tiles_per_wg;
  const int64_t t1 = (t0 + a.tiles_per_wg < T) ? t0 + a.tiles_per_wg : T;
  unsigned* const sync = a.sync + (size_t)b * 2;
  f32x4 cf[NCH][8];
  load_coef<NCH>(a, b, half, cf);
  __shared__ __attribute__((aligned(16))) f32x4 sCfT[2 * NCH * 8];
  const f32x4* cfl = nullptr;
  if constexpr (AttnCfl<NCH, false>::value) cfl = attn_cf_table<NCH>(cf, sCfT);
  attn_pass1<NCH>(a, b, part, t0, t1, cf, cfl);
  attn_group_barrier(sync, P, a.status);
  attn_pass2<NCH>(a, b, part, P, t0, t1, cf, nullptr, cfl);
  attn_group_barrier(sync, P, a.status);
  const int C = NCH * 32;
  if (tid < 64) {
    double a1 = 0.0, a2 = 0.0;
    for (int u = 0; u < P; ++u) {
      const float* cp = a.ch_part + ((size_t)b * P + u) * C * 2;
      for (int c = tid; c < C; c += 64) {
        a1 += (double)attn_peer_load(cp + c * 2, 1);
        a2 += (double)attn_peer_load(cp + c * 2 + 1, 1);
      }
    }
#pragma unroll
    for (int m = 32; m >= 1; m >>= 1) {
      a1 += __shfl_xor(a1, m, 64);
      a2 += __shfl_xor(a2, m, 64);
    }
    if (tid == 0) {
      const double cnt = (double)a.vox * C;
      const double mu = a1 / cnt;
      double var = a2 / cnt - mu * mu;
      var = var < 0.0 ? 0.0 : var;
      sTot[0] = mu;
      sTot[1] = 1.0 / sqrt(var + 1e-5);
    }
  }
  __syncthreads();
  if (tid < C) {
    const float sc = (float)sTot[1] * a.out_gamma[tid];
    sOut[tid][0] = sc;
    sOut[tid][1] = a.out_beta[tid] - (float)sTot[0] * sc;
  }
  __syncthreads();
  float* const yb = a.y + (size_t)b * a.vox * C;
  const float* const xb = a.x + (size_t)b * a.vox * C;
  const int64_t v0 = t0 * 32, v1 = t1 * 32 < a.vox ? t1 * 32 : a.vox;
  for (int64_t i = v0 * C / 4 + tid; i < v1 * C / 4; i += 512) {
    const int c = (int)((i * 4) % C);
    const f32x4 y = ((const f32x4*)yb)[i], x = ((const f32x4*)xb)[i];
    f32x4 o;
#pragma unroll
    for (int e = 0; e < 4; ++e) o[e] = sOut[c + e][0] * y[e] + sOut[c + e][1] + x[e];
    ((f32x4*)yb)[i] = o;
  }
}

int tiles_per_wg_for(int64_t vox, int nsplit) {
  const int64_t T = (vox + 31) / 32;
  int64_t per = (T + nsplit - 1) / nsplit;
  per = (per + 7) / 8 * 8;
  return (int)per;
}

}

int attn_fused_nsplit_for(int64_t vox, int batch) {
  const int64_t T = (vox + 31) / 32;
  static const int target = getenv("CD_ATTN_WGS") ? atoi(getenv("CD_ATTN_WGS")) : 256;
  int64_t want = (target + batch - 1) / batch;
  const int64_t cap = (T + 15) / 16;
  int64_t n = want < cap ? want : cap;
  if (n < 1) n = 1;
  if (n > 128) n = 128;
  const int per = tiles_per_wg_for(vox, (int)n);
  n = (T + per - 1) / per;
  return (int)n;
}

bool attn_moments_eligible(int C) { return C == 32; }
size_t attn_moment_floats(int batch, int nsplit) { return (size_t)batch * nsplit * ATTN_MOM; }

void launch_attn_kv_context(const float* x, int C, const float* coef, const void* wqkv_f16x2, float* partials, int batch,
                            int64_t vox, int nsplit, hipStream_t s, const GnDefer* defer, int* status, float* moments) {
  CD_REQUIRE(C == 32 || C == 64 || C == 96 || C == 128, "fused attention: 32..128 input channels");
  CD_REQUIRE(!moments || attn_moments_eligible(C), "fused attention: the moment form takes 32 channels");
  AttnArgs a{};
  a.mom = moments;
  a.status = status;
  a.x = x; a.coef = coef; a.wqkv = (const u32x4*)wqkv_f16x2; a.C = C; a.vox = vox; a.tiles_per_wg = tiles_per_wg_for(vox, nsplit);
  a.partials = partials; a.nsplit = nsplit;
  if (defer) a.defer = *defer;
  char cat[64];
  std::snprintf(cat, sizeof cat, "attn_kv_context C%d n%ld", C, (long)vox);
  prof::Scope scope(cat, s, 2.0 * ((moments ? 3.0 : 2.0) * C + (moments ? 64 : 32)) * 32 * (double)vox * batch,
                    4.0 * batch * (double)vox * C);
  const dim3 grid((unsigned)nsplit, (unsigned)batch);
  if (moments) {
    hipLaunchKernelGGL((attn_kv_context_kernel<1, true>), grid, dim3(512), 0, s, a);
    CD_HIP(hipGetLastError());
    return;
  }
  switch (C / 32) {
    case 1: hipLaunchKernelGGL((attn_kv_context_kernel<1, false>), grid, dim3(512), 0, s, a); break;
    case 2: hipLaunchKernelGGL((attn_kv_context_kernel<2, false>), grid, dim3(512), 0, s, a); break;
    case 3: hipLaunchKernelGGL((attn_kv_context_kernel<3, false>), grid, dim3(512), 0, s, a); break;
    default: hipLaunchKernelGGL((attn_kv_context_kernel<4, false>), grid, dim3(512), 0, s, a); break;
  }
  CD_HIP(hipGetLastError());
}

void launch_attn_out(const float* x, int C, const float* coef, const void* wqkv_f16x2, const float* wT_b, const float* bias,
                     float* y, float* ch_part, int batch, int64_t vox, int nsplit, hipStream_t s, const GnDefer* defer,
                     const float* partials, const float* w_out, float scale, int* status, const float* moments,
                     const float* out_gamma, const float* out_beta) {
  CD_REQUIRE(C == 32 || C == 64 || C == 96 || C == 128, "fused attention: 32..128 channels");
  CD_REQUIRE(!moments || (attn_moments_eligible(C) && !wT_b && out_gamma && out_beta && (vox * C) % 4 == 0),
             "fused attention: the moment form folds the weights itself and needs the closing GroupNorm's parameters");
  AttnArgs a{};
  a.mom = const_cast<float*>(moments); a.out_gamma = out_gamma; a.out_beta = out_beta;
  a.status = status;
  a.x = x; a.coef = coef; a.wqkv = (const u32x4*)wqkv_f16x2; a.C = C; a.vox = vox; a.tiles_per_wg = tiles_per_wg_for(vox, nsplit);
  a.wT = wT_b; a.bias = bias; a.y = y; a.ch_part = ch_part;
  CD_REQUIRE(wT_b || (partials && w_out), "attn_out: folded weights or the pass-1 partials to fold them from");
  a.partials = const_cast<float*>(partials); a.nsplit = nsplit; a.fold_wout = w_out; a.fold_scale = scale;
  if (defer) a.defer = *defer;
  char cat[64];
  std::snprintf(cat, sizeof cat, "attn_out C%d n%ld", C, (long)vox);
  prof::Scope scope(cat, s, 2.0 * (2.0 * C) * 32 * (double)vox * batch, 4.0 * batch * (double)vox * C * 2);
  const dim3 grid((unsigned)nsplit, (unsigned)batch);
  if (moments) {
    hipLaunchKernelGGL((attn_out_kernel<1, true>), grid, dim3(512), 0, s, a);
    CD_HIP(hipGetLastError());
    return;
  }
  switch (C / 32) {
    case 1: hipLaunchKernelGGL((attn_out_kernel<1, false>), grid, dim3(512), 0, s, a); break;
    case 2: hipLaunchKernelGGL((attn_out_kernel<2, false>), grid, dim3(512), 0, s, a); break;
    case 3: hipLaunchKernelGGL((attn_out_kernel<3, false>), grid, dim3(512), 0, s, a); break;
    default: hipLaunchKernelGGL((attn_out_kernel<4, false>), grid, dim3(512), 0, s, a); break;
  }
  CD_HIP(hipGetLastError());
}

bool attn_small_eligible(int64_t vox) {
  static const int max_vox = getenv("CD_ATTN_SMALL_MAX") ? atoi(getenv("CD_ATTN_SMALL_MAX")) : 1024;
  return vox <= max_vox;
}
void launch_attn_small(const float* x, int C, const float* coef, const void* wqkv_f16x2, float* partials, const float* w_out,
                       float scale, const float* bias, const float* out_gamma, const float* out_beta, float* y, float* ch_part,
                       int batch, int64_t vox, hipStream_t s, const GnDefer* defer, int* status, int max_parts, unsigned* coop_sync) {
  CD_REQUIRE(C == 32 || C == 64 || C == 96 || C == 128, "fused attention: 32..128 channels");
  CD_REQUIRE((vox * C) % 4 == 0, "fused attention: whole float4 rows");
  AttnArgs a{};
  a.status = status;
  a.x = x; a.coef = coef; a.wqkv = (const u32x4*)wqkv_f16x2; a.C = C; a.vox = vox; a.tiles_per_wg = tiles_per_wg_for(vox, 1);
  a.partials = partials; a.nsplit = 1; a.wT = nullptr; a.fold_wout = w_out; a.fold_scale = scale; a.bias = bias;
  a.y = y; a.ch_part = ch_part; a.out_gamma = out_gamma; a.out_beta = out_beta;
  if (defer) a.defer = *defer;
  char cat[64];
  std::snprintf(cat, sizeof cat, "attn_small C%d n%ld", C, (long)vox);
  prof::Scope scope(cat, s, 2.0 * (4.0 * C + 32) * 32 * (double)vox * batch, 4.0 * batch * (double)vox * C * 3);
  static const int coop_env = getenv("CD_ATTN_COOP") ? atoi(getenv("CD_ATTN_COOP")) : 0;
  const int64_t T = (vox + 31) / 32;
  int P = coop_env < max_parts ? coop_env : max_parts;
  while (P > 1 && ((int64_t)batch * P > 256 || T < 4 * P)) --P;
  if (P > 1 && batch % 8 == 0 && status && coop_sync) {
    int per = (int)((T + P - 1) / P);
    while (P > 1 && (int64_t)(P - 1) * per >= T) { --P; per = (int)((T + P - 1) / P); }
    if (P > 1) {
      CD_REQUIRE(batch <= kAttnCoopSamples, "attention: batch too large for the co-operative form");
      CD_HIP(hipMemsetAsync(coop_sync, 0, sizeof(unsigned) * 2 * batch, s));
      a.sync = coop_sync; a.coop = 1; a.nsplit = P; a.tiles_per_wg = per;
      const dim3 cgrid((unsigned)(batch * P));
      switch (C / 32) {
        case 1: hipLaunchKernelGGL(attn_coop_kernel<1>, cgrid, dim3(512), 0, s, a); break;
        case 2: hipLaunchKernelGGL(attn_coop_kernel<2>, cgrid, dim3(512), 0, s, a); break;
        case 3: hipLaunchKernelGGL(attn_coop_kernel<3>, cgrid, dim3(512), 0, s, a); break;
        default: hipLaunchKernelGGL(attn_coop_kernel<4>, cgrid, dim3(512), 0, s, a); break;
      }
      CD_HIP(hipGetLastError());
      return;
    }
  }
  const dim3 grid((unsigned)batch);
  switch (C / 32) {
    case 1: hipLaunchKernelGGL(attn_small_kernel<1>, grid, dim3(512), 0, s, a); break;
    case 2: hipLaunchKernelGGL(attn_small_kernel<2>, grid, dim3(512), 0, s, a); break;
    case 3: hipLaunchKernelGGL(attn_small_kernel<3>, grid, dim3(512), 0, s, a); break;
    default: hipLaunchKernelGGL(attn_small_kernel<4>, grid, dim3(512), 0, s, a); break;
  }
  CD_HIP(hipGetLastError());
}

}
```

### calodiffusion_amd/csrc/ops.hip

```cpp
#include "plan_internal.h"

namespace cd {

__global__ void to_cl_kernel(const float* __restrict__ src, float* __restrict__ dst, int channels, int64_t vox) {
  const int b = blockIdx.y;
  const int64_t total = vox * channels;
  for (int64_t i = (int64_t)blockIdx.x * 256 + threadIdx.x; i < total; i += (int64_t)gridDim.x * 256) {
    const int c = (int)(i % channels);
    const int64_t v = i / channels;
    dst[(size_t)b * total + i] = src[(size_t)b * total + (size_t)c * vox + v];
  }
}
__global__ void to_planar_kernel(const float* __restrict__ src, float* __restrict__ dst, int channels, int64_t vox) {
  const int b = blockIdx.y;
  const int64_t total = vox * channels;
  for (int64_t i = (int64_t)blockIdx.x * 256 + threadIdx.x; i < total; i += (int64_t)gridDim.x * 256) {
    const int64_t v = i % vox;
    const int c = (int)(i / vox);
    dst[(size_t)b * total + i] = src[(size_t)b * total + (size_t)v * channels + c];
  }
}
static void launch_transpose_to_cl(const float* ncdhw, float* ndhwc, int batch, int channels, int64_t vox, hipStream_t s) {
  int64_t bx = (vox * channels + 255) / 256;
  if (bx > 1024) bx = 1024;
  hipLaunchKernelGGL(to_cl_kernel, dim3((unsigned)bx, batch), dim3(256), 0, s, ncdhw, ndhwc, channels, vox);
  CD_HIP(hipGetLastError());
}
static void launch_transpose_to_planar(const float* ndhwc, float* ncdhw, int batch, int channels, int64_t vox, hipStream_t s) {
  int64_t bx = (vox * channels + 255) / 256;
  if (bx > 1024) bx = 1024;
  hipLaunchKernelGGL(to_planar_kernel, dim3((unsigned)bx, batch), dim3(256), 0, s, ndhwc, ncdhw, channels, vox);
  CD_HIP(hipGetLastError());
}

}

extern "C" {

static AbsmaxWords op_absmax_words(Arena& ws, hipStream_t s) {
  constexpr size_t kWords = 8;
  unsigned* w = ws.get<unsigned>(kWords);
  CD_HIP(hipMemsetAsync(w, 0, sizeof(unsigned) * kWords, s));
  return AbsmaxWords{w, w + kWords};
}
size_t cd_op_scratch_bytes(int batch, int max_channels, int64_t max_voxels) {
  return (size_t)256 * 256 * 64 * 4 * 4 + (size_t)batch * 64 * 64 * 16 + (size_t)batch * max_channels * max_voxels * 4 + (1 << 20);
}

int cd_op_to_channels_last(const float* ncdhw, float* ndhwc, int batch, int channels, int64_t voxels, void* stream) {
  return guarded([&] { launch_transpose_to_cl(ncdhw, ndhwc, batch, channels, voxels, (hipStream_t)stream); });
}
int cd_op_to_ncdhw(const float* ndhwc, float* ncdhw, int batch, int channels, int64_t voxels, void* stream) {
  return guarded([&] { launch_transpose_to_planar(ndhwc, ncdhw, batch, channels, voxels, (hipStream_t)stream); });
}

int cd_op_cyl_conv(const float* x0, int c0, const float* x1, int c1, const float* w, const float* bias, float* y,
                   int batch, int cout, const int32_t dims_in[3], const int32_t kernel[3], const int32_t stride[3],
                   void* scratch, void* stream) {
  return guarded([&] {
    CD_REQUIRE(x0 && w && y && scratch, "null argument");
    hipStream_t s = (hipStream_t)stream;
    const int taps = kernel[0] * kernel[1] * kernel[2];
    float* wpk = (float*)scratch;
    launch_pack_weights(w, wpk, cout, c0 + c1, taps, false, s);
    const Dims3 din{dims_in[0], dims_in[1], dims_in[2]};
    if (taps == 1) {
      PointwiseArgs a;
      a.in0 = x0; a.ld0 = c0; a.c0 = c0; a.in1 = x1; a.ld1 = c1; a.c1 = c1; a.wpk = wpk; a.bias = bias; a.out = y;
      a.batch = batch; a.cout = cout; a.vox = din.vox();
      launch_pointwise(a, s);
    } else {
      CD_REQUIRE(cout % 32 == 0, "cout must be a multiple of 32");
      ConvGeom g;
      g.in = din;
      g.kd = kernel[0]; g.kh = kernel[1]; g.kw = kernel[2]; g.sz = stride[0]; g.sh = stride[1]; g.sw = stride[2];
      g.out = Dims3{(din.d + 2 - g.kd) / g.sz + 1, (din.h + 2 - g.kh) / g.sh + 1, (din.w + 2 - g.kw) / g.sw + 1};
      ConvFusion fu;
      if (taps == 27 || taps == 48) {
        float* w3 = wpk + packed_weight_floats(c0 + c1, cout, taps);
        launch_pack_weights_split16(w, w3, cout, c0 + c1, taps, s);
        fu.wpk_bf16x3 = w3;
      }
      launch_conv_mfma(x0, c0, x1, c1, wpk, bias, y, batch, cout, g, s, fu);
    }
  });
}

int cd_op_zslide_conv(const float* x, int cin, const float* w, const float* bias, float* y, float* ch_part, int* units, int batch,
                      int cout, const int32_t dims[3], int chunks, void* scratch, void* stream) {
  return guarded([&] {
    CD_REQUIRE(x && w && y && ch_part && units && scratch && chunks >= 0, "bad argument");
    CD_REQUIRE(cin % 32 == 0 && cout % 32 == 0, "channel counts must be multiples of 32");
    hipStream_t s = (hipStream_t)stream;
    launch_pack_weights_f16x2(w, scratch, cout, cin, 27, s);
    const Dims3 d{dims[0], dims[1], dims[2]};
    ConvGeom g{d, d, 3, 3, 3, 1, 1, 1};
    ConvFusion fu;
    int u = 0;
    fu.act = 1; fu.ch_part = ch_part; fu.units = &u; fu.zs_chunks = chunks;
    CD_REQUIRE(try_launch_conv_zslide(x, cin, nullptr, 0, scratch, bias, y, batch, cout, g, s, fu) && u > 0,
               "this grid is not eligible for the z-slide kernel");
    *units = u;
  });
}

int cd_op_cyl_conv_transpose(const float* x, const float* w, const float* bias, float* y, int batch, int channels,
                             const int32_t dims_in[3], int kernel_z, int stride_z, const int32_t out_pad[3],
                             void* scratch, void* stream) {
  return guarded([&] {
    CD_REQUIRE(x && w && y && scratch, "null argument");
    CD_REQUIRE(out_pad[0] == 0, "z output padding is always 0 (models.py:339)");
    hipStream_t s = (hipStream_t)stream;
    float* wpk = (float*)scratch;
    launch_pack_weights(w, wpk, channels, channels, kernel_z * 16, true, s);
    float* wpk16 = wpk + ((packed_weight_floats(channels, channels, kernel_z * 16) + 63) & ~(size_t)63);
    launch_pack_weights_f16x2(w, wpk16, channels, channels, kernel_z * 16, s, true, false);
    const Dims3 din{dims_in[0], dims_in[1], dims_in[2]};
    const Dims3 dout{(din.d - 1) * stride_z - 2 + kernel_z, 2 * din.h + out_pad[1], 2 * din.w + out_pad[2]};
    launch_conv_transpose_mfma(x, channels, wpk, bias, y, batch, channels, din, dout, kernel_z, stride_z, s, wpk16, nullptr);
  });
}

int cd_op_init_conv(const float* x_ncdhw, const float* w, const float* bias, float* y, int batch, int cin, int cout,
                    const int32_t dims[3], void* scratch, void* stream) {
  return guarded([&] {
    CD_REQUIRE(x_ncdhw && w && y && scratch, "null argument");
    hipStream_t s = (hipStream_t)stream;
    float* wpk = (float*)scratch;
    launch_pack_init_weights(w, wpk, cout, cin, s);
    InitConvArgs a;
    a.x = x_ncdhw; a.cx = cin; a.cin = cin; a.wpk = wpk; a.bias = bias; a.out = y; a.batch = batch; a.cout = cout;
    a.dims = Dims3{dims[0], dims[1], dims[2]};
    launch_init_conv(a, s);
  });
}

int cd_op_init_pair_conv(const float* x, const float* w0, const float* b0, const float* w1, const float* b1, int cin, const float* r_w,
                         const float* z_d, const float* phi_h, int use_rz, int use_phi, const float* scale_b, float* y, float* ch_part,
                         int* units, int batch, const int32_t dims[3], int slabs, void* scratch, void* stream) {
  return guarded([&] {
    CD_REQUIRE(x && w0 && w1 && y && ch_part && units && scratch && batch > 0 && slabs >= 0, "bad argument");
    CD_REQUIRE(cin == 1 + 2 * (use_rz ? 1 : 0) + (use_phi ? 1 : 0), "cin must be 1 + the coordinate channels in use");
    CD_REQUIRE(cin == 1 || (r_w && z_d && phi_h), "coordinate channels need their profiles");
    hipStream_t s = (hipStream_t)stream;
    const Dims3 d{dims[0], dims[1], dims[2]};
    CD_REQUIRE(init_pair_eligible(d), "this grid is not eligible for the composed init pair");
    auto up = [](size_t n) { return (n + 63) & ~(size_t)63; };
    float* wpk0 = (float*)scratch;
    float* tab0 = wpk0 + up((size_t)27 * cin * 32);
    float* wc = tab0 + up((size_t)d.vox() * 32);
    float* tab1 = wc + up(kInitPairWeightBytes / 4);
    launch_pack_init_weights(w0, wpk0, 32, cin, s);
    InitConvArgs a;
    a.cin = cin; a.cx = 1; a.wpk = wpk0; a.bias = b0; a.cout = 32; a.dims = d; a.use_rz = use_rz; a.use_phi = use_phi;
    a.r_w = r_w; a.z_d = z_d; a.phi_h = phi_h; a.coord_table = tab0;
    launch_init_coord_table(a, s);
    launch_init_pair_build(w0, cin, w1, b1, tab0, wc, tab1, d, s);
    InitPairArgs ia;
    ia.x = x; ia.scale_b = scale_b; ia.wc = wc; ia.table = tab1; ia.out = y; ia.ch_part = ch_part; ia.batch = batch; ia.dims = d;
    ia.slabs = slabs;
    launch_init_pair_conv(ia, units, s);
  });
}

int cd_op_group_norm(const float* x, float* y, const float* gamma, const float* beta, int batch, int channels,
                     int64_t voxels, int groups, int silu, const float* add_bc, const float* residual,
                     void* scratch, void* stream) {
  return guarded([&] {
    CD_REQUIRE(x && y && gamma && beta && scratch, "null argument");
    hipStream_t s = (hipStream_t)stream;
    const int ns = gn_nsplit_for(voxels, batch);
    float* part = (float*)scratch;
    float* coef = part + (size_t)batch * ns * channels * 2;
    launch_ch_stats(x, part, batch, channels, voxels, ns, s);
    launch_gn_finalize(part, ns, gamma, beta, add_bc, channels, coef, batch, channels, groups, voxels, s);
    launch_gn_apply(x, y, coef, batch, channels, voxels, silu, residual, nullptr, 0, nullptr, s);
  });
}

int cd_op_resnet_block(const float* x0, int c0, const float* x1, int c1, const float* const* w, const float* cond, float* y,
                       int batch, int cout, const int32_t dims[3], int groups, void* workspace, size_t workspace_bytes,
                       void* stream) {
  return guarded([&] {
    CD_REQUIRE(x0 && w && y && workspace, "null argument");
    hipStream_t s = (hipStream_t)stream;
    const int cin = c0 + c1;
    Arena ws;
    ws.reset((char*)workspace, workspace_bytes, false);
    float* p1 = ws.get<float>(packed_weight_floats(cin, cout, 27));
    float* p2 = ws.get<float>(packed_weight_floats(cout, cout, 27));
    launch_pack_weights(w[0], p1, cout, cin, 27, false, s);
    launch_pack_weights(w[4], p2, cout, cout, 27, false, s);
    float* q1 = ws.get<float>(packed_split16_bytes(cin, cout, 27) / 4);
    float* q2 = ws.get<float>(packed_split16_bytes(cout, cout, 27) / 4);
    launch_pack_weights_split16(w[0], q1, cout, cin, 27, s);
    launch_pack_weights_split16(w[4], q2, cout, cout, 27, s);
    ResP r;
    r.cin = cin; r.cout = cout; r.has_res = w[10] != nullptr;
    r.c1w3 = q1; r.c2w3 = q2;
    r.c1w = p1; r.c1b = w[1]; r.n1g = w[2]; r.n1b = w[3]; r.c2w = p2; r.c2b = w[5]; r.n2g = w[6]; r.n2b = w[7];
    if (r.has_res) {
      float* p3 = ws.get<float>(packed_weight_floats(cin, cout, 1));
      launch_pack_weights(w[10], p3, cout, cin, 1, false, s);
      r.rw = p3; r.rb = w[11];
    }
    if (w[8] && cond) {
      float* emb = ws.get<float>((size_t)batch * cout);
      launch_silu_linear(cond, w[8], w[9], emb, batch, 128, cout, s);
      r.emb = emb; r.emb_ld = cout;
    }
    Run run{&ws, s, batch, groups};
    const Dims3 d{dims[0], dims[1], dims[2]};
    float* out = res_block(run, r, x0, c0, x1, c1, d);
    CD_HIP(hipMemcpyAsync(y, out, sizeof(float) * (size_t)batch * d.vox() * cout, hipMemcpyDeviceToDevice, s));
  });
}

int cd_op_linear_attention(const float* x, const float* const* w, float* y, int batch, int channels, const int32_t dims[3],
                           void* workspace, size_t workspace_bytes, void* stream) {
  return guarded([&] {
    CD_REQUIRE(x && w && y && workspace, "null argument");
    hipStream_t s = (hipStream_t)stream;
    Arena ws;
    ws.reset((char*)workspace, workspace_bytes, false);
    float* pq = ws.get<float>(packed_weight_floats(channels, 96, 1));
    launch_pack_weights(w[2], pq, 96, channels, 1, false, s);
    float* pq16 = ws.get<float>(packed_f16x2_bytes(channels, 96, 1) / 4);
    launch_pack_weights_f16x2(w[2], pq16, 96, channels, 1, s);
    AttnP a;
    a.c = channels; a.ng = w[0]; a.nb = w[1]; a.qkv = pq; a.ow = w[3]; a.ob = w[4]; a.gg = w[5]; a.gb = w[6];
    a.qkv16 = pq16;
    Run run{&ws, s, batch, 8};
    const Dims3 d{dims[0], dims[1], dims[2]};
    float* out = attn_block(run, a, x, d);
    CD_HIP(hipMemcpyAsync(y, out, sizeof(float) * (size_t)batch * d.vox() * channels, hipMemcpyDeviceToDevice, s));
  });
}

int cd_op_conv_backward(const float* x0, int c0, const float* x1, int c1, const float* w, const float* dy, float* dx, float* dw,
                        float* db, int batch, int cout, const int32_t dims_in[3], const int32_t kernel[3],
                        const int32_t stride[3], void* workspace, size_t workspace_bytes, void* stream) {
  return guarded([&] {
    CD_REQUIRE(x0 && w && dy && dw && workspace, "null argument");
    Arena ws;
    ws.reset((char*)workspace, workspace_bytes, false);
    Run run{&ws, (hipStream_t)stream, batch, 8};
    run.amax = op_absmax_words(ws, run.s);
    ConvGeom g;
    g.in = Dims3{dims_in[0], dims_in[1], dims_in[2]};
    g.kd = kernel[0]; g.kh = kernel[1]; g.kw = kernel[2]; g.sz = stride[0]; g.sh = stride[1]; g.sw = stride[2];
    if (g.kd * g.kh * g.kw == 1) g.out = g.in;
    else g.out = Dims3{(g.in.d + 2 - g.kd) / g.sz + 1, (g.in.h + 2 - g.kh) / g.sh + 1, (g.in.w + 2 - g.kw) / g.sw + 1};
    conv_backward(run, x0, c0, x1, c1, w, dy, dx, dw, db, cout, g);
  });
}

int cd_op_conv_transpose_backward(const float* x, const float* w, const float* dy, float* dx, float* dw, float* db, int batch,
                                  int channels, const int32_t dims_in[3], int kernel_z, int stride_z, const int32_t out_pad[3],
                                  void* workspace, size_t workspace_bytes, void* stream) {
  return guarded([&] {
    CD_REQUIRE(x && w && dy && dw && workspace, "null argument");
    Arena ws;
    ws.reset((char*)workspace, workspace_bytes, false);
    Run run{&ws, (hipStream_t)stream, batch, 8};
    run.amax = op_absmax_words(ws, run.s);
    const Dims3 din{dims_in[0], dims_in[1], dims_in[2]};
    const Dims3 dout{(din.d - 1) * stride_z - 2 + kernel_z, 2 * din.h + out_pad[1], 2 * din.w + out_pad[2]};
    conv_transpose_backward(run, x, w, dy, dx, dw, db, channels, din, dout, kernel_z, stride_z);
  });
}

int cd_op_group_norm_backward(const float* x, const float* gamma, const float* beta, const float* dy, float* dx, float* dgamma,
                              float* dbeta, float* dadd, int batch, int channels, int64_t voxels, int groups, int silu,
                              void* workspace, size_t workspace_bytes, void* stream) {
  return guarded([&] {
    CD_REQUIRE(x && gamma && beta && dy && dx && dgamma && dbeta && workspace, "null argument");
    hipStream_t s = (hipStream_t)stream;
    Arena ws;
    ws.reset((char*)workspace, workspace_bytes, false);
    Run run{&ws, s, batch, groups};
    int units = 0;
    float* part = stats_pass(run, x, channels, voxels, &units);
    float* coef = ws.get<float>((size_t)batch * channels * 4);
    float* stat = ws.get<float>((size_t)batch * groups * 2);
    launch_gn_finalize(part, units, gamma, beta, nullptr, 0, coef, batch, channels, groups, voxels, s, stat);
    float* scratch = ws.get<float>(gn_backward_scratch_floats(batch, channels, voxels));
    launch_gn_backward(dy, x, coef, stat, gamma, dx, dgamma, dbeta, dadd, channels, batch, channels, voxels, groups, silu, scratch,
                       false, s);
  });
}

}
```

### calodiffusion_amd/csrc/plan_internal.h

```cpp
#pragma once
#include "arena.h"
#include "guarded.h"
#include "kernels_bwd.h"
#include "kernels_conv.h"
#include "kernels_embed_head.h"
#include "kernels_geom.h"
#include "kernels_gn.h"
#include "kernels_sampler.h"
#include "kernels_wgrad.h"
#include "kernels_widen.h"

#include <map>
#include <string>
#include <vector>

namespace cd {

enum PackKind { PK_NONE = 0, PK_CONV = 1, PK_CONVT = 2, PK_INIT = 3 };
struct WeightEntry {
  std::string name;
  int64_t numel = 0;
  int64_t src_numel = 0;
  size_t raw_off = 0;
  PackKind pack = PK_NONE;
// ... 57 lines not shown

}

using namespace cd;

struct CdPlan {
  CdUnetDesc desc{};
  int cfg_sizes[CD_MAX_SIZES] = {};
  int nres = 0;
  std::vector<Dims3> shapes;
  std::vector<int> up_kz;
  std::vector<Dims3> up_out;
  std::vector<WeightEntry> weights;
  std::map<std::string, int> index;
  float* arena = nullptr;
  size_t arena_floats = 0;

  int init_w = -1, init_b = -1, head_w = -1, head_b = -1;
  int tw[3] = {-1, -1, -1}, tb[3] = {-1, -1, -1}, cw[3] = {-1, -1, -1}, cb[3] = {-1, -1, -1};
  std::vector<LevelW> downs, ups;
  ResW mid1, mid2, fin;
  AttnW mid_attn;
  int emb_ld = 0;
  EmbedLayer* d_embed_layers = nullptr;
  int n_embed_layers = 0;
  std::vector<std::pair<int, int>> embed_list;

  float* d_coords = nullptr;
  float* d_init_table = nullptr;
  bool coords_set = false;
  void* d_pair_w = nullptr;
  float* d_pair_table = nullptr;
  bool init_pair_ready = false;

  static constexpr int kMaxSteps = 4096;
  static constexpr int kEmbedChunk = 16;
  float* d_table = nullptr;
  int* d_counter = nullptr;
  float* d_stepvals = nullptr;
  int* status_word = nullptr;

  hipStream_t cap_stream = nullptr;
  std::vector<PackJob> pack_jobs;
  PackJob* d_pack_jobs = nullptr;
  size_t dg_floats = 0;
  std::vector<PackJob> dg_jobs;
  PackJob* d_dg_jobs = nullptr;
  const float* dg_jobs_at = nullptr;
  const float* dg_images = nullptr;
  DgImg dg(int i) const {
    DgImg g;
    const WeightEntry& w = weights[i];
    if (dg_images && w.dg_mode) {
      g.pk = dg_images + w.dg_pk_off;
      if (w.dg_mode != 1) g.pk3 = dg_images + w.dg_pk3_off;
    }
    return g;
  }
  unsigned* d_attn_sync = nullptr;
  StepGraph ddim_graph, prog_graph;

  size_t grad_floats = 0;
  std::vector<LinearWgradJob> lin_jobs_host;
  LinearWgradJob* d_lin_jobs = nullptr;

  struct FlatEmbed {
    const CdRadialMap* map = nullptr;
    const float* enc_w = nullptr;
    const float* dec_w = nullptr;
    const CdGeomMap* genc = nullptr;
    const CdGeomMap* gdec = nullptr;
    bool want_grads = true;
    int64_t state() const { return map ? (int64_t)map->V : (int64_t)genc->layers * genc->cols; }
    size_t grad_floats() const {
      const size_t n = map ? (size_t)map->wtotal : (want_grads ? (size_t)genc->layers * genc->rows * genc->cols : 0);
      return (n + 63) & ~(size_t)63;
    }
  } fe;
  const FlatEmbed* flat() const { return (fe.map || fe.genc) ? &fe : nullptr; }
  int64_t state_per() const { return flat() ? fe.state() : shapes[0].vox(); }
  size_t embed_grad_floats() const { return flat() ? fe.grad_floats() : 0; }
  size_t enc_grad_off() const { return grad_floats; }
  size_t dec_grad_off() const { return grad_floats + embed_grad_floats(); }

  bool widened = false;
  std::vector<WidenJob> expand_jobs, fold_jobs;
  WidenJob *d_expand_jobs = nullptr, *d_fold_jobs = nullptr;
  size_t wide_grad_floats = 0;

  Arena ws;

  const float* raw(int i) const { return arena + weights[i].raw_off; }
  const float* packed(int i) const { return arena + weights[i].pk_off; }
  const void* packed3(int i) const { return weights[i].pk3_off ? (const void*)(arena + weights[i].pk3_off) : nullptr; }
};

namespace cd {

struct Run {
  Arena* ws;
  hipStream_t s;
  int B;
  int groups;
  int* status = nullptr;
  GnParamQueue* gq = nullptr;
  WgradReduceQueue* wq = nullptr;
  std::vector<float*> wq_held;
  AbsmaxWords amax;
  bool param_grads = true;
  bool dry() const { return ws->dry(); }
  unsigned* amax_word() { return dry() ? nullptr : amax.take(); }
  float* wgrad_part(size_t floats) {
    float* part = ws->get<float>(floats);
    if (wq) wq_held.push_back(part);
    return part;
  }
  void release_wgrad_part(float* part) {
    if (!wq) ws->release(part);
  }
  WgradAux wgrad_aux(const unsigned* gmax = nullptr, const unsigned* xmax = nullptr) {
    WgradAux a;
    a.queue = wq; a.words = &amax; a.gmax = gmax; a.xmax = xmax;
    return a;
  }
};

struct ResP {
  int cin = 0, cout = 0;
  bool has_res = false;
  const float *c1w = nullptr, *c1b = nullptr, *n1g = nullptr, *n1b = nullptr;
  const void *c1w3 = nullptr, *c2w3 = nullptr;
  const float *c2w = nullptr, *c2b = nullptr, *n2g = nullptr, *n2b = nullptr;
  const float *rw = nullptr, *rb = nullptr;
  const void* rw16 = nullptr;
  const float* emb = nullptr;
  int emb_ld = 0;
};
struct AttnP {
  int c = 0;
  const float *ng = nullptr, *nb = nullptr, *qkv = nullptr, *ow = nullptr, *ob = nullptr, *gg = nullptr, *gb = nullptr;
  const void* qkv16 = nullptr;
  unsigned* coop_sync = nullptr;
};

ResP resolve(const CdPlan* p, const ResW& w, const float* emb);
AttnP resolve(const CdPlan* p, const AttnW& w);

struct FwdOpts {
  float* emb_pre = nullptr;
  float* scal_pre = nullptr;
  const HeadArgs* upd = nullptr;
};

struct LazyClose;
float* stats_pass(Run& r, const float* x, int C, int64_t vox, int* units);
float* conv3_with_stats(Run& r, const float* x0, int c0, const float* x1, int c1, const float* wpk, const void* wpk3,
                        const float* bias, float* out, int cout, Dims3 dims, const float* coef_in, int* units,
                        const GnDefer* defer_in = nullptr, float* coef_buf = nullptr, const ConvFusion::GnOut* gn_out = nullptr);
struct ConvDone {
  float* h1 = nullptr;
  float* part = nullptr;
  int units = 0;
};
float* res_block(Run& r, const ResP& w, const float* x0, int c0, const float* x1, int c1, Dims3 dims,
                 float** part_out = nullptr, int* units_out = nullptr, LazyClose* lazy = nullptr, float* h1_side = nullptr,
                 const ConvDone* h1_done = nullptr);
float* attn_block(Run& r, const AttnP& w, const float* x, Dims3 dims, float* xpart = nullptr, int xunits = 0);
void bias_grad(Run& r, const float* dy, int C, int64_t vox, float* db);
void conv_backward(Run& r, const float* x0, int c0, const float* x1, int c1, const float* w_raw, const float* dy, float* dx,
                   float* dw, float* db, int cout, const ConvGeom& g, const DgImg* img = nullptr, const float* xcoef = nullptr,
                   const float* dx_add = nullptr, int* dx_added = nullptr, const unsigned* dy_max = nullptr);
void conv_transpose_backward(Run& r, const float* x, const float* w_raw, const float* dy, float* dx, float* dw, float* db, int c,
                             Dims3 din, Dims3 dout, int kz, int sz, const DgImg* img = nullptr);
EmbedArgs embed_args(CdPlan* p, int B, const float* cond, const float* t, int kind, float* emb, float* scal);
void forward_impl(CdPlan* p, int B, const float* x, const float* cond, const float* t, float* out, bool raw, hipStream_t s,
                  const FwdOpts* opt = nullptr);
inline void launch_embed_in(const CdPlan::FlatEmbed& e, const float* x, const float* scal, float* g, int batch, hipStream_t s) {
  if (e.map) radial_embed_in(e.map, e.enc_w, x, scal, g, batch, s);
  else geom_embed_in(e.genc, x, scal, g, batch, s);
}
inline void launch_embed_out(const CdPlan::FlatEmbed& e, const float* F, const float* x, const float* scal, int objective, float* out,
                             const HeadArgs* upd, int batch, hipStream_t s) {
  if (e.map) radial_embed_out(e.map, e.dec_w, F, x, scal, objective, out, upd, batch, s);
  else geom_embed_out(e.gdec, F, x, scal, objective, out, upd, batch, s);
}
inline void launch_embed_dec_vjp(const CdPlan::FlatEmbed& e, const float* F, const float* gf, float* dF, float* dd, int batch,
                                 hipStream_t s) {
  if (e.map) radial_embed_dec_vjp(e.map, e.dec_w, F, gf, dF, dd, batch, s);
  else geom_embed_dec_vjp(e.gdec, F, gf, dF, dd, batch, s);
}
inline void launch_embed_enc_vjp(const CdPlan::FlatEmbed& e, const float* x, const float* dg, const float* gy, const float* scal,
                                 int objective, float* dx, float* dw, int batch, hipStream_t s) {
  if (e.map) radial_embed_enc_vjp(e.map, e.enc_w, x, dg, gy, scal, objective, dx, dw, batch, s);
  else geom_embed_enc_vjp(e.genc, x, dg, gy, scal, objective, dx, dw, batch, s);
}
void check_ready(CdPlan* p, bool need_coords);
void dgrad_images(CdPlan* p);
void denoise_vjp_impl(CdPlan* p, int B, const float* x, const float* sigma, const float* cond, const float* gy, float* dx, float* grads,
                      bool param_grads, hipStream_t s);

template <typename F>
size_t dry_forward_bytes(CdPlan* plan, int batch, F&& front) {
  struct Restore {
    ~Restore() { set_conv_precision_override(-1); }
  } restore;
  size_t need = 0;
  for (int mode : {(int)PREC_F16X2, (int)PREC_BF16X3, (int)PREC_F32}) {
    set_conv_precision_override(mode);
    plan->ws.reset(nullptr, 0, true);
    front();
    forward_impl(plan, batch, nullptr, nullptr, nullptr, nullptr, false, nullptr);
    need = plan->ws.high() > need ? plan->ws.high() : need;
  }
  return need;
}

template <typename F>
bool run_with_range_fallback(CdPlan* plan, hipStream_t s, F&& run, bool report_sticky = true) {
  struct Restore {
    CdPlan* p;
    ~Restore() {
      p->status_word = p->d_counter + 2;
      set_conv_precision_override(-1);
    }
  } restore{plan};
  plan->status_word = plan->d_counter + 3;
  CD_HIP(hipMemsetAsync(plan->d_counter + 3, 0, sizeof(int), s));
  run(false);
  if (conv_precision() != PREC_F16X2) return false;
  int flags = 0;
  CD_HIP(hipMemcpyAsync(&flags, plan->d_counter + 3, sizeof(int), hipMemcpyDeviceToHost, s));
  CD_HIP(hipStreamSynchronize(s));
  if (!(flags & 1)) return false;
  set_conv_precision_override(PREC_BF16X3);
  run(true);
  if (report_sticky) launch_or_word(plan->d_counter + 2, 2, s);
  return true;
}

}
```

### calodiffusion_amd/engine.py

```python
from __future__ import annotations

import ctypes as C
import os

import numpy as np
import torch

from .abi import (CD_ABI_VERSION, CD_MAX_SIZES, EXPORTED_SYMBOLS, LIB_PATH, LOSS_TYPES, OBJECTIVES, SOP_DENOISE, SOP_DENOISE_PS,
                  SOP_LINCOMB, SOP_LINDIV, SOP_RANDN, SOP_RECORD, TIME_KINDS, CdClassifierDesc, CdGeneratorRun, CdHlfDesc,
                  CdLayerMlpDesc, CdSamplerOp, CdStep, CdUnetDesc, WorkspaceCache, _P, _SIGNATURES, _check,
                  _check_built_from_these_sources, _dev32, _i32x3, _ptr, _stream, get_conv_precision, load_library, profile_begin,
                  profile_end, randn, require_gpu, set_conv_precision)
from .ops import Ops


def _sigma_b(sigma, B: int) -> torch.Tensor:
    sigma = _dev32(sigma, "sigma").reshape(-1)
    if sigma.numel() == 1 and B > 1:
        sigma = sigma.expand(B).contiguous()
    return sigma


def _pack_ops(program) -> np.ndarray:
    ops = np.zeros((len(program.ops), C.sizeof(CdSamplerOp) // 4), dtype=np.int32)
# ... 58 lines not shown

    def __init__(self, unet, rz_input=False, phi_input=False, time_kind="raw", objective="hybrid", sigma_data=1.0,
                 coords=None):
        self.lib = load_library()
        self.device_name = require_gpu()
        self.unet = unet
        d = self.desc = unet_desc(unet, rz_input, phi_input, time_kind, objective, sigma_data)
        self.grid = tuple(unet.grid)
        self.voxels = int(np.prod(self.grid))
        handle = _P()
        _check(self.lib.cd_plan_create(C.byref(d), C.byref(handle)))
        self.plan = handle
        self._weights_version = None
        self._weight_order = None
        self._weight_ids = None
        self._held_weights = []
        self._ws = WorkspaceCache()
        self._grad_layout = None
        self.range_fallbacks = 0
        self.embedding = None
        self._rmap = self._enc_flat = self._dec_flat = self._gmaps = self._embed_version = None
        self.state_shape = (1,) + self.grid
        self.device = next(unet.parameters()).device
        if self.device.type != "cuda":
            raise RuntimeError("move the model to the GPU first (model.to('cuda')): calodiffusion_amd has no CPU path")
        if coords is not None:
            r, z, phi = (np.ascontiguousarray(a, dtype=np.float32) for a in coords)
            assert len(r) == self.grid[2] and len(z) == self.grid[0] and len(phi) == self.grid[1]
            _check(self.lib.cd_plan_set_coords(self.plan, r.ctypes.data, z.ctypes.data, phi.ctypes.data, _stream()))
        self.sync_weights(force=True)

    @classmethod
    def for_unet(cls, unet):
        opts = getattr(unet, "_engine_opts", {})
        return cls(unet, **opts)

    def __del__(self):
        try:
            if getattr(self, "plan", None):
                self.lib.cd_plan_destroy(self.plan)
                self.plan = None
        except Exception:
            pass

    def _version(self):
        ps = list(self.unet.parameters())
        return tuple(p._version for p in ps) + tuple(p.data_ptr() for p in ps) + (tuple(id(p) for p in ps),)

    def _plan_weights(self):
        n = C.c_int()
        _check(self.lib.cd_plan_num_weights(self.plan, C.byref(n)))
        buf = C.create_string_buffer(256)
        numel = C.c_int64()
        out = []
        for i in range(n.value):
            _check(self.lib.cd_plan_weight_name(self.plan, i, buf, 256, C.byref(numel)))
            out.append((buf.value.decode(), numel.value))
        return out

    def set_embedding(self, nn_embed):
        from .hgcal import HGCalConverter
        self._grad_layout = None
        self._ws.clear()
        self._embed_version = None
        self._rmap = self._enc_flat = self._dec_flat = self._gmaps = None
        if nn_embed is None:
            _check(self.lib.cd_plan_set_radial(self.plan, None, None, None, 0, _stream()))
            self.embedding, self.state_shape = None, (1,) + self.grid
            return
        if isinstance(nn_embed, HGCalConverter):
            have = (nn_embed.num_layers, nn_embed.num_alpha_bins, nn_embed.num_r_bins)
            if have != self.grid:
                raise ValueError(f"the embedding maps onto the grid {have}, the U-Net runs on {self.grid}")
            if nn_embed.norm:
                raise ValueError("an in-model HGCalConverter has no norm (the reference calls init(norm=pre_embed), "
                                 "calodiffusion.py:117): bind a converter initialised with norm=False")
            self.embedding, self.state_shape = nn_embed, (1, have[0], int(nn_embed.embeder.mat.shape[-1]))
        else:
            rmap = nn_embed.gc.radial_map()
            if (rmap.L, rmap.A, rmap.R) != self.grid:
                raise ValueError(f"the embedding maps onto the grid {(rmap.L, rmap.A, rmap.R)}, the U-Net runs on {self.grid}")
            self._rmap = rmap
            self._enc_flat = torch.empty(rmap.wtotal, dtype=torch.float32, device=self.device)
            self._dec_flat = torch.empty(rmap.wtotal, dtype=torch.float32, device=self.device)
            self.embedding, self.state_shape = nn_embed, (rmap.V,)
        self._sync_embedding()

    def _check_state(self, x, name, what="x"):
        if tuple(x.shape[1:]) != self.state_shape:
            raise ValueError(f"{name}: {what} has shape {tuple(x.shape)}, expected (B,) + {self.state_shape}")

    def _embed_is_geom(self) -> bool:
        return self.embedding is not None and self._rmap is None

    def _embed_params(self):
        if self._embed_is_geom():
            return [(f"NN_embed.{k}", p) for k, p in self.embedding.named_parameters()]
        return ([(f"NN_embed.encs.{i}", lay.weight) for i, lay in enumerate(self.embedding.encs)] +
                [(f"NN_embed.decs.{i}", lay.weight) for i, lay in enumerate(self.embedding.decs)])

    def embedding_trains(self) -> bool:
        return self.embedding is not None and any(p.requires_grad for _, p in self._embed_params())

    def _sync_embedding(self):
        if self._embed_is_geom():
            enc, dec = self.embedding.embeder.packed(), self.embedding.decoder.packed()
            ver = (enc.handle.value, dec.handle.value, self.embedding_trains())
            if ver != self._embed_version:
                _check(self.lib.cd_plan_set_geom(self.plan, enc.handle, dec.handle, int(ver[-1]), _stream()))
                self._gmaps = (enc, dec)
                self._grad_layout = None
                self._ws.drop("train", "vjp")
                self._embed_version = ver
            return
        ps = [p for _, p in self._embed_params()]
        ver = tuple(p._version for p in ps) + tuple(p.data_ptr() for p in ps) + (self.embedding_trains(),)
        if ver == self._embed_version:
            return
        n = len(self.embedding.encs)
        torch.cat([p.detach().reshape(-1).to(device=self.device, dtype=torch.float32) for p in ps[:n]], out=self._enc_flat)
        torch.cat([p.detach().reshape(-1).to(device=self.device, dtype=torch.float32) for p in ps[n:]], out=self._dec_flat)
        if self._embed_version is None or self._embed_version[-1] != ver[-1]:
            _check(self.lib.cd_plan_set_radial(self.plan, self._rmap.handle, self._enc_flat.data_ptr(), self._dec_flat.data_ptr(),
                                               int(ver[-1]), _stream()))
        self._embed_version = ver

    def sync_weights(self, force=False):
        if self.embedding is not None:
            self._sync_embedding()
        ver = self._version()
        if not force and ver == self._weights_version:
            return
        ids = ver[-1]
        if self._weight_order is None or self._weight_ids != ids:
            sd = self.unet.state_dict(keep_vars=True)
            order = []
            for name, numel in self._plan_weights():
                if name not in sd:
                    raise RuntimeError(f"state_dict has no tensor named {name!r}")
                if sd[name].numel() != numel:
                    raise RuntimeError(f"{name}: {sd[name].numel()} elements, HIP plan expects {numel}")
                order.append((name, sd[name]))
            missing = set(sd) - {name for name, _ in order}
            if missing:
                raise RuntimeError(f"HIP plan does not consume these state_dict tensors: {sorted(missing)[:5]} ...")
            self._weight_order, self._weight_ids = order, ids
        tensors = [_dev32(t.detach(), name) for name, t in self._weight_order]
        ptrs = (_P * len(tensors))(*[t.data_ptr() for t in tensors])
        _check(self.lib.cd_plan_set_weights(self.plan, len(tensors), ptrs, _stream()))
        self._held_weights = tensors
        self._weights_version = ver

    _WS_SWITCHES = ("CD_NO_DEEP_LEVEL", "CD_NO_PW_CLOSE", "CD_NO_FUSED_ATTN", "CD_NO_GNDEFER", "CD_ATTN_COMBINE_LAUNCH", "CD_PW_F32",
                    "CD_NO_ATTN_MOMENTS", "CD_ATTN_MOM_MIN", "CD_NO_DEEP_SIDE_CONV")

    def _ws_key(self, batch: int):
        return (int(batch),) + tuple(os.environ.get(k) for k in self._WS_SWITCHES)

    def workspace(self, batch: int) -> torch.Tensor:
        return self._ws.get("net", self._ws_key(batch), self.device,
                            lambda: _nbytes(self.lib.cd_plan_workspace_bytes, self.plan, batch))

    def unet_forward(self, x, cond, time):
        x, cond, time = _dev32(x, "x"), _dev32(cond, "cond"), _dev32(time, "time")
        B = x.shape[0]
        if tuple(x.shape[1:]) != (self.unet.channels,) + self.grid:
            raise ValueError(f"x has shape {tuple(x.shape)}, expected (B, {self.unet.channels}, {self.grid})")
        if self.desc.cond_sin:
            if cond.numel() != B:
                raise ValueError("cond_embed='sin' takes cond of shape (B,)")
        elif cond.shape != (B, self.unet.cond_size):
            raise ValueError("cond must be (B, cond_size)")
        if time.numel() != B:
            raise ValueError("time must be (B,)")
        self.sync_weights()
        ws = self.workspace(B)
        out = torch.empty((B, 1) + self.grid, dtype=torch.float32, device=x.device)
        _check(self.lib.cd_unet_forward(self.plan, B, x.data_ptr(), cond.data_ptr(), time.data_ptr(), out.data_ptr(),
                                        ws.data_ptr(), ws.numel(), _stream()))
        return out

    safe_denoise = True

    def denoise(self, x, sigma, cond):
        x, cond = _dev32(x, "x"), _dev32(cond, "cond")
        B = x.shape[0]
        sigma = _sigma_b(sigma, B)
        if tuple(x.shape[1:]) != self.state_shape or sigma.numel() != B or cond.shape != (B, self.unet.cond_size):
            raise ValueError(f"denoise shapes: x {tuple(x.shape)} (expected (B,) + {self.state_shape}), sigma {tuple(sigma.shape)}, "
                             f"cond {tuple(cond.shape)}")
        self.sync_weights()
        ws = self.workspace(B)
        out = torch.empty_like(x)
        if self.safe_denoise:
            fell = C.c_int(0)
            _check(self.lib.cd_denoise_safe(self.plan, B, x.data_ptr(), sigma.data_ptr(), cond.data_ptr(), out.data_ptr(),
                                            ws.data_ptr(), ws.numel(), C.byref(fell), _stream()))
            if fell.value:
                self.range_fallbacks += 1
        else:
            _check(self.lib.cd_denoise(self.plan, B, x.data_ptr(), sigma.data_ptr(), cond.data_ptr(), out.data_ptr(),
                                       ws.data_ptr(), ws.numel(), _stream()))
        return out

    def ddim_sample(self, start, cond, steps: np.ndarray, step_noise=None, seed=0, offset=0, debug=False, use_graph=True,
                    out=None, noise_stride=0):
        start, cond = _dev32(start, "start"), _dev32(cond, "cond")
        B = start.shape[0]
        self._check_state(start, "ddim_sample", "start")
        steps = np.ascontiguousarray(steps, dtype=np.float32)
        n_steps = steps.shape[0]
        assert steps.shape == (n_steps, 4)
        self.sync_weights()
        ws = self.workspace(B)
        x_out = torch.empty_like(start) if out is None else out
        xs, x0s = _trajectories(start, n_steps, debug, debug, zeroed=False)
        if step_noise is not None:
            step_noise = _dev32(step_noise, "step_noise")
            assert step_noise.shape[0] == n_steps and step_noise[0].numel() == start.numel()
        _check(self.lib.cd_ddim_sample(self.plan, B, start.data_ptr(), cond.data_ptr(),
                                       steps.ctypes.data_as(C.POINTER(CdStep)), n_steps, _ptr(step_noise), int(seed),
                                       int(offset), int(noise_stride), x_out.data_ptr(), _ptr(xs), _ptr(x0s),
                                       int(bool(use_graph)), ws.data_ptr(), ws.numel(), _stream()))
        self.check_status()
        return x_out, xs, x0s

    def sampler_run(self, start, cond, program, step_noise=None, seed=0, offset=0, noise_stride=0, debug=False, use_graph=True):
        start, cond = _dev32(start, "start"), _dev32(cond, "cond")
        B = start.shape[0]
        self._check_state(start, "sampler_run", "start")
        coefs = np.ascontiguousarray(program.coefs, dtype=np.float32)
        n_steps, n_coef = coefs.shape
        ops = _pack_ops(program)
        op_begin = None
        if program.op_begin is not None:
            assert len(program.op_begin) == n_steps + 1
            op_begin = (C.c_int32 * (n_steps + 1))(*program.op_begin)
        self.sync_weights()
        ws = self._ws.get("sampler", self._ws_key(B), self.device,
                          _nbytes(self.lib.cd_plan_sampler_workspace_bytes, self.plan, B, program.n_bufs, n_steps, n_coef))
        x_out = torch.empty_like(start)
        xs, x0s, step_noise = _program_io(start, program, n_steps, step_noise, debug, "(B,1,D,H,W)")
        _check(self.lib.cd_sampler_run(self.plan, B, start.data_ptr(), float(program.start_scale), cond.data_ptr(), program.n_bufs,
                                       n_steps, ops.ctypes.data_as(C.POINTER(CdSamplerOp)), len(program.ops), op_begin,
                                       coefs.ctypes.data, n_coef, _ptr(step_noise), int(seed), int(offset), int(noise_stride),
                                       x_out.data_ptr(), _ptr(xs), _ptr(x0s), int(bool(use_graph)), ws.data_ptr(), ws.numel(), _stream()))
        self.check_status()
        return x_out, xs, x0s

    def check_status(self):
        flags = C.c_int(0)
        _check(self.lib.cd_plan_status(self.plan, C.byref(flags), _stream()))
        if flags.value & 2:
            self.range_fallbacks += 1
        if flags.value & 1:
            raise FloatingPointError("calodiff: an activation exceeded the fp16 range of the f16x2 convolution kernels "
                                     "(outputs contain inf/NaN); set CD_CONV_PRECISION=bf16x3 for the full fp32 range")

    def grad_layout(self):
        if self._grad_layout is None:
            off, total = C.c_int64(), C.c_int64()
            weights = self._plan_weights()
            lay = {}
            for i, (name, numel) in enumerate(weights):
                _check(self.lib.cd_plan_grad_layout(self.plan, i, C.byref(off), C.byref(total)))
                lay[name] = (off.value, numel)
            if self.embedding is not None and (not self._embed_is_geom() or self.embedding_trains()):
                sizes = ((self._rmap.wtotal,) * 2 if not self._embed_is_geom() else
                         (self.embedding.embeder.mat.numel(), self.embedding.decoder.mat.numel()))
                for k, name in enumerate(("NN_embed.encs", "NN_embed.decs")):
                    _check(self.lib.cd_plan_grad_layout(self.plan, len(weights) + k, C.byref(off), C.byref(total)))
                    lay[name] = (off.value, sizes[k])
            self._grad_layout = (lay, total.value)
        return self._grad_layout

    def train_workspace(self, batch: int) -> torch.Tensor:
        return self._ws.get("train", self._ws_key(batch), self.device,
                            lambda: _nbytes(self.lib.cd_plan_train_workspace_bytes, self.plan, batch))

    def _loss_io(self, data, noise, sigma, cond, name):
        data, noise, cond = _dev32(data, "data"), _dev32(noise, "noise"), _dev32(cond, "cond")
        sigma = _dev32(sigma, "sigma").reshape(-1)
        B = data.shape[0]
        self._check_state(data, name, "data")
        if noise.shape != data.shape or sigma.numel() != B:
            raise ValueError(f"{name}: noise {tuple(noise.shape)} must have data's shape and sigma {tuple(sigma.shape)} B elements")
        return data, noise, sigma, cond, B

    def train_step(self, data, noise, sigma, cond, loss_type="l2"):
        data, noise, sigma, cond, B = self._loss_io(data, noise, sigma, cond, "train_step")
        self.sync_weights()
        ws = self.train_workspace(B)
        _, total = self.grad_layout()
        flat = torch.empty(total, dtype=torch.float32, device=data.device)
        loss = torch.empty((), dtype=torch.float64, device=data.device)
        _check(self.lib.cd_train_step(self.plan, B, data.data_ptr(), noise.data_ptr(), sigma.data_ptr(), cond.data_ptr(),
                                      LOSS_TYPES[loss_type], loss.data_ptr(), flat.data_ptr(), ws.data_ptr(), ws.numel(), _stream()))
        return loss, flat

    def vjp_workspace(self, batch: int, with_param_grads: bool) -> torch.Tensor:
        mode = bool(with_param_grads)
        return self._ws.get("vjp", self._ws_key(batch) + (mode,), self.device,
                            lambda: _nbytes(self.lib.cd_plan_vjp_workspace_bytes, self.plan, batch, int(mode)))

    def denoise_vjp(self, x, sigma, cond, gy, param_grads: bool):
        x, cond, gy = _dev32(x, "x"), _dev32(cond, "cond"), _dev32(gy, "gy")
        B = x.shape[0]
# ... 231 lines not shown
```

### calodiffusion_amd/ops.py

```python
from __future__ import annotations

import ctypes as C
from typing import Dict

import numpy as np
import torch

from .abi import WorkspaceCache, _P, _check, _dev32, _i32x3, _ptr, _stream, load_library, require_gpu


class Ops:

    def __init__(self):
        self.lib = load_library()
        require_gpu()
        self._ws = WorkspaceCache()

    def scratch(self, batch, channels, voxels):
        return self._ws.get("scratch", (), "cuda", self.lib.cd_op_scratch_bytes(batch, channels, voxels))

    def to_channels_last(self, x):
        x = _dev32(x, "x")
        B, Cc = x.shape[:2]
        vox = int(np.prod(x.shape[2:]))
# ... 7 lines not shown
        vox = int(np.prod(y.shape[1:-1]))
        x = torch.empty((B, Cc) + tuple(y.shape[1:-1]), dtype=torch.float32, device=y.device)
        _check(self.lib.cd_op_to_ncdhw(y.data_ptr(), x.data_ptr(), B, Cc, vox, _stream()))
        return x

    def cyl_conv(self, x_cl, w, bias, stride=(1, 1, 1), x1_cl=None):
        x_cl, w = _dev32(x_cl, "x"), _dev32(w, "w")
        B, D, H, W, c0 = x_cl.shape
        c1 = 0 if x1_cl is None else x1_cl.shape[-1]
        cout = w.shape[0]
        k = tuple(w.shape[2:])
        if k == (1, 1, 1):
            od = (D, H, W)
        else:
            od = ((D + 2 - k[0]) // stride[0] + 1, (H + 2 - k[1]) // stride[1] + 1, (W + 2 - k[2]) // stride[2] + 1)
        y = torch.empty((B,) + od + (cout,), dtype=torch.float32, device=x_cl.device)
        sc = self.scratch(B, max(c0 + c1, cout), D * H * W)
        _check(self.lib.cd_op_cyl_conv(x_cl.data_ptr(), c0, _ptr(x1_cl), c1, w.data_ptr(), _ptr(bias), y.data_ptr(), B, cout,
                                       _i32x3((D, H, W)), _i32x3(k), _i32x3(stride), sc.data_ptr(), _stream()))
        return y

    def zslide_conv_chunked(self, x_cl, w, bias, chunks=0):
        x_cl, w = _dev32(x_cl, "x"), _dev32(w, "w")
        B, D, H, W, cin = x_cl.shape
        cout = w.shape[0]
        y = torch.empty((B, D, H, W, cout), dtype=torch.float32, device=x_cl.device)
        cap = (D * H * W + 31) // 32
        part = torch.zeros((B, cap, cout, 2), dtype=torch.float32, device=x_cl.device)
        units = C.c_int()
        sc = self.scratch(B, max(cin, cout), D * H * W)
        _check(self.lib.cd_op_zslide_conv(x_cl.data_ptr(), cin, w.data_ptr(), _ptr(bias), y.data_ptr(), part.data_ptr(), C.byref(units),
                                          B, cout, _i32x3((D, H, W)), int(chunks), sc.data_ptr(), _stream()))
        u = units.value
        return y, part.view(-1)[:B * u * cout * 2].view(B, u, cout, 2).double().sum(1)

    def cyl_conv_transpose(self, x_cl, w, bias, kernel_z, stride_z, out_pad):
        x_cl, w = _dev32(x_cl, "x"), _dev32(w, "w")
        B, D, H, W, c = x_cl.shape
        od = ((D - 1) * stride_z - 2 + kernel_z, 2 * H + out_pad[1], 2 * W + out_pad[2])
        y = torch.empty((B,) + od + (c,), dtype=torch.float32, device=x_cl.device)
        sc = self.scratch(B, c, int(np.prod(od)))
        _check(self.lib.cd_op_cyl_conv_transpose(x_cl.data_ptr(), w.data_ptr(), _ptr(bias), y.data_ptr(), B, c,
                                                 _i32x3((D, H, W)), kernel_z, stride_z, _i32x3(out_pad), sc.data_ptr(),
                                                 _stream()))
        return y

    def init_conv(self, x_ncdhw, w, bias):
        x, w = _dev32(x_ncdhw, "x"), _dev32(w, "w")
        B, cin, D, H, W = x.shape
        cout = w.shape[0]
        y = torch.empty((B, D, H, W, cout), dtype=torch.float32, device=x.device)
        sc = self.scratch(B, cout, D * H * W)
        _check(self.lib.cd_op_init_conv(x.data_ptr(), w.data_ptr(), _ptr(bias), y.data_ptr(), B, cin, cout, _i32x3((D, H, W)),
                                        sc.data_ptr(), _stream()))
        return y

    def init_pair_conv(self, x, w0, b0, w1, b1, profiles=None, scale=None, slabs=0, y=None, part=None):
        x, w0, w1 = _dev32(x, "x"), _dev32(w0, "w0"), _dev32(w1, "w1")
        B, D, H, W = x.shape
        cin = w0.shape[1]
        if y is None:
            y = torch.empty((B, D, H, W, 32), dtype=torch.float32, device=x.device)
        if part is None:
            part = torch.zeros((B * D * 64,), dtype=torch.float32, device=x.device)
        r_w, z_d, phi_h, use_rz, use_phi = profiles if profiles is not None else (None, None, None, 0, 0)
        units = C.c_int()
        sc = self.scratch(B, 32, D * H * W)
        _check(self.lib.cd_op_init_pair_conv(x.data_ptr(), w0.data_ptr(), _ptr(b0), w1.data_ptr(), _ptr(b1), cin, _ptr(r_w), _ptr(z_d),
                                             _ptr(phi_h), int(use_rz), int(use_phi), _ptr(scale), y.data_ptr(), part.data_ptr(),
                                             C.byref(units), B, _i32x3((D, H, W)), int(slabs), sc.data_ptr(), _stream()))
        u = units.value
        return y, part.view(-1)[:B * u * 64].view(B, u, 32, 2).double().sum(1), u

    def group_norm(self, x_cl, gamma, beta, groups, silu=False, add_bc=None, residual=None):
        x = _dev32(x_cl, "x")
        B, Cc = x.shape[0], x.shape[-1]
        vox = int(np.prod(x.shape[1:-1]))
        y = torch.empty_like(x)
        sc = self.scratch(B, Cc, vox)
        _check(self.lib.cd_op_group_norm(x.data_ptr(), y.data_ptr(), gamma.data_ptr(), beta.data_ptr(), B, Cc, vox, groups,
                                         int(silu), _ptr(add_bc), _ptr(residual), sc.data_ptr(), _stream()))
        return y

    def _bws(self, nbytes=1 << 30):
        return self._ws.get("bwd", (), "cuda", nbytes)

    def conv_backward(self, x_cl, w, dy_cl, stride=(1, 1, 1), x1_cl=None, need_dx=True, bias=True):
        x, w, dy = _dev32(x_cl, "x"), _dev32(w, "w"), _dev32(dy_cl, "dy")
        B, D, H, W, c0 = x.shape
        c1 = 0 if x1_cl is None else x1_cl.shape[-1]
        cout, k = w.shape[0], tuple(w.shape[2:])
        dx = torch.empty((B, D, H, W, c0 + c1), dtype=torch.float32, device=x.device) if need_dx else None
        dw = torch.empty_like(w)
        db = torch.empty((cout,), dtype=torch.float32, device=x.device) if bias else None
        ws = self._bws()
        _check(self.lib.cd_op_conv_backward(x.data_ptr(), c0, _ptr(x1_cl), c1, w.data_ptr(), dy.data_ptr(), _ptr(dx), dw.data_ptr(),
                                            _ptr(db), B, cout, _i32x3((D, H, W)), _i32x3(k), _i32x3(stride), ws.data_ptr(),
                                            ws.numel(), _stream()))
        return dx, dw, db

    def conv_transpose_backward(self, x_cl, w, dy_cl, kernel_z, stride_z, out_pad):
        x, w, dy = _dev32(x_cl, "x"), _dev32(w, "w"), _dev32(dy_cl, "dy")
        B, D, H, W, c = x.shape
        dx, dw = torch.empty_like(x), torch.empty_like(w)
        db = torch.empty((c,), dtype=torch.float32, device=x.device)
        ws = self._bws()
        _check(self.lib.cd_op_conv_transpose_backward(x.data_ptr(), w.data_ptr(), dy.data_ptr(), dx.data_ptr(), dw.data_ptr(),
                                                      db.data_ptr(), B, c, _i32x3((D, H, W)), kernel_z, stride_z, _i32x3(out_pad),
                                                      ws.data_ptr(), ws.numel(), _stream()))
        return dx, dw, db

    def group_norm_backward(self, x_cl, gamma, beta, dy_cl, groups, silu=False, want_dadd=False):
        x, dy = _dev32(x_cl, "x"), _dev32(dy_cl, "dy")
        B, Cc = x.shape[0], x.shape[-1]
        vox = int(np.prod(x.shape[1:-1]))
        dx, dg, db = torch.empty_like(x), torch.empty_like(gamma), torch.empty_like(beta)
        dadd = torch.empty((B, Cc), dtype=torch.float32, device=x.device) if want_dadd else None
        ws = self._bws()
        _check(self.lib.cd_op_group_norm_backward(x.data_ptr(), gamma.data_ptr(), beta.data_ptr(), dy.data_ptr(), dx.data_ptr(),
                                                  dg.data_ptr(), db.data_ptr(), _ptr(dadd), B, Cc, vox, groups, int(silu),
                                                  ws.data_ptr(), ws.numel(), _stream()))
        return dx, dg, db, dadd

    _RES_KEYS = ("block1.proj.conv.weight", "block1.proj.conv.bias", "block1.norm.weight", "block1.norm.bias",
                 "block2.proj.conv.weight", "block2.proj.conv.bias", "block2.norm.weight", "block2.norm.bias",
                 "mlp.1.weight", "mlp.1.bias", "res_conv.conv.weight", "res_conv.conv.bias")

    def resnet_block(self, x_cl, sd: Dict[str, torch.Tensor], cond=None, groups=8, x1_cl=None):
        x = _dev32(x_cl, "x")
        B, D, H, W, c0 = x.shape
        c1 = 0 if x1_cl is None else x1_cl.shape[-1]
        cout = sd["block1.proj.conv.weight"].shape[0]
        ptrs = (_P * 12)(*[(sd[k].data_ptr() if k in sd else None) for k in self._RES_KEYS])
        y = torch.empty((B, D, H, W, cout), dtype=torch.float32, device=x.device)
        nbytes = self.lib.cd_op_scratch_bytes(B, max(c0 + c1, cout), D * H * W) + 4 * B * D * H * W * cout * 4 * 4
        ws = torch.empty(nbytes, dtype=torch.uint8, device=x.device)
        _check(self.lib.cd_op_resnet_block(x.data_ptr(), c0, _ptr(x1_cl), c1, ptrs, _ptr(cond), y.data_ptr(), B, cout,
                                           _i32x3((D, H, W)), groups, ws.data_ptr(), ws.numel(), _stream()))
        return y

    _ATTN_KEYS = ("fn.norm.weight", "fn.norm.bias", "fn.fn.to_qkv.conv.weight", "fn.fn.to_out.0.conv.weight",
                  "fn.fn.to_out.0.conv.bias", "fn.fn.to_out.1.weight", "fn.fn.to_out.1.bias")

    def linear_attention(self, x_cl, sd: Dict[str, torch.Tensor]):
        x = _dev32(x_cl, "x")
        B, D, H, W, c = x.shape
        ptrs = (_P * 7)(*[sd[k].data_ptr() for k in self._ATTN_KEYS])
        y = torch.empty_like(x)
        nbytes = self.lib.cd_op_scratch_bytes(B, 96, D * H * W) + 4 * B * D * H * W * 96 * 4
        ws = torch.empty(nbytes, dtype=torch.uint8, device=x.device)
        _check(self.lib.cd_op_linear_attention(x.data_ptr(), ptrs, y.data_ptr(), B, c, _i32x3((D, H, W)), ws.data_ptr(),
                                               ws.numel(), _stream()))
        return y
```

### include/calodiff.h

```cpp
#ifndef CALODIFF_H
#define CALODIFF_H

#include <stddef.h>
#include <stdint.h>

#ifdef __cplusplus
extern "C" {
#endif

#define CD_OK 0
#define CD_EINVAL -1
#define CD_EHIP -2
#define CD_ENOGPU -3
#define CD_EWEIGHTS -4
#define CD_EWORKSPACE -5

#define CD_MAX_SIZES 8

#define CD_ABI_VERSION 3

#define CD_TIME_LOG 0
#define CD_TIME_SIGMA 1
#define CD_TIME_RAW 2

// ... 163 lines not shown
  int32_t objective;
  float sigma_data;
} CdLayerMlpDesc;

int cd_layer_forward(const CdLayerMlpDesc* desc, const float* const* weights, int n_weights, int batch, const float* x,
                     const float* cond, const float* time, float* out, void* stream);
int cd_layer_denoise(const CdLayerMlpDesc* desc, const float* const* weights, int n_weights, int batch, const float* x,
                     const float* sigma, const float* cond, float* out, void* stream);
int cd_layer_sample(const CdLayerMlpDesc* desc, const float* const* weights, int n_weights, int batch, const float* start,
                    const float* cond, const CdStep* steps_dev, int n_steps, const float* step_noise, float* x_out, float* xs,
                    float* x0s, void* stream);
int cd_layer_sampler_run(const CdLayerMlpDesc* desc, const float* const* weights, int n_weights, int batch, const float* start,
                         float start_scale, const float* cond, int n_bufs, int n_steps, const CdSamplerOp* ops_dev, int n_ops,
                         const int32_t* op_begin_dev, const float* coefs_dev, int n_coef, const float* step_noise, uint64_t seed,
                         uint64_t offset, uint64_t noise_stride, float* x_out, float* xs, float* x0s, void* stream);

int cd_layer_train_workspace_bytes(const CdLayerMlpDesc* desc, int batch, size_t* bytes);
int cd_layer_train_step(const CdLayerMlpDesc* desc, const float* const* weights, int n_weights, int batch, const float* data,
                        const float* noise, const float* sigma, const float* cond, double* loss_out, float* grads,
                        void* workspace, size_t workspace_bytes, void* stream);
int cd_layer_train_step_loss(const CdLayerMlpDesc* desc, const float* const* weights, int n_weights, int batch, const float* data,
                             const float* noise, const float* sigma, const float* cond, int loss_type ,
                             double* loss_out, float* grads, void* workspace, size_t workspace_bytes, void* stream);
int cd_layer_loss(const CdLayerMlpDesc* desc, const float* const* weights, int n_weights, int batch, const float* data,
                  const float* noise, const float* sigma, const float* cond, int loss_type , double* loss_out,
                  void* workspace, size_t workspace_bytes, void* stream);

int cd_layer_vjp_workspace_bytes(const CdLayerMlpDesc* desc, int batch, int with_param_grads, size_t* bytes);
int cd_layer_denoise_vjp(const CdLayerMlpDesc* desc, const float* const* weights, int n_weights, int batch, const float* x,
                         const float* sigma, const float* cond, const float* gy, float* dx, float* grads ,
                         void* workspace, size_t workspace_bytes, void* stream);

typedef struct CdGenerator CdGenerator;
int cd_generator_create(const void* blob, size_t bytes, CdGenerator** out, void* stream);
int cd_generator_destroy(CdGenerator* gen);
int cd_generator_checksum(const void* data, size_t bytes, uint64_t* out);
int cd_generator_info(const CdGenerator* gen, int32_t* info);
int cd_generator_geometry(const CdGenerator* gen, int32_t* geom);
int cd_generator_workspace_bytes(CdGenerator* gen, int batch, size_t* bytes);
int cd_generator_run(CdGenerator* gen, int batch, const float* energy, int energy_is_normalised, const float* layers ,
                     uint64_t seed, uint64_t offset, int first_row, int global_batch, float* showers, float* layers_out ,
                     uint64_t* next_offset , void* workspace, size_t workspace_bytes, void* stream);

struct CdGeneratorRun {
  uint32_t struct_size;
  int32_t batch;
  const float* energy;
  int32_t energy_is_normalised;
  int32_t sparse_mode;
  const float* layers;
  uint64_t seed, offset;
  int32_t first_row, global_batch;
  float* showers;
  float* layers_out;
  uint64_t* next_offset;
  uint64_t decode_seed, decode_offset;
  uint64_t* next_decode_offset;
  void* workspace;
  size_t workspace_bytes;
  void* stream;
};
typedef struct CdGeneratorRun CdGeneratorRun;
int cd_generator_run_ex(CdGenerator* gen, const CdGeneratorRun* args);

struct CdHlfDesc {
  uint32_t struct_size;
  int32_t n_layers;
  const int32_t* layer_offset;
  const double* eta;
  const double* phi;
  const int32_t* with_centres;
};
typedef struct CdHlfDesc CdHlfDesc;
typedef struct CdHlf CdHlf;
int cd_hlf_create(const CdHlfDesc* desc, CdHlf** out, void* stream);
int cd_hlf_destroy(CdHlf* hlf);
int cd_hlf_compute(const CdHlf* hlf, const float* showers, int batch, float threshold, double* out, int32_t* n_hits, void* stream);

#define CD_FPD_MAX_D 256
#define CD_FPD_SLICE_ROWS 2048
size_t cd_fpd_workspace_bytes(int d, int sets, int max_count);
int cd_fpd_moments(const double* x, int64_t rows, int d, const double* centre, const int32_t* idx, int64_t idx_stride,
                   const int32_t* counts , int sets, double* mean, double* cov, int32_t* status, void* workspace,
                   size_t workspace_bytes, void* stream);

#define CD_KPD_BLOCK 64
#define CD_KPD_MAX_COUNT 1048576
size_t cd_kpd_workspace_bytes(int sets, int max_count);
int cd_kpd_sums(const double* x, int64_t rows, int d, const int32_t* idx, int64_t idx_stride, const int32_t* counts ,
                int sets, double gamma, int degree, double* sums, int32_t* status, void* workspace, size_t workspace_bytes,
                void* stream);
#define CD_HIST_CHUNK_ROWS 256
#define CD_HIST_MAX_EDGES 64
size_t cd_column_histograms_workspace_bytes(int64_t row_count, int d, int nedges);
int cd_column_histograms(const double* x, int64_t row_begin, int64_t row_count, int d, const double* edges, int nedges,
                         uint32_t* counts, void* workspace, size_t workspace_bytes, void* stream);

#define CD_CLS_MAX_DIM 4096
#define CD_CLS_MAX_LAYERS 8
#define CD_CLS_MAX_BATCH 256
#define CD_CLS_MAX_ROWS_PER_CALL 65536
typedef struct CdClassifierDesc {
  uint32_t struct_size;
  int32_t input_dim;
  int32_t hidden;
  int32_t num_layer;
  float negative_slope;
  float dropout_p;
} CdClassifierDesc;
int cd_classifier_num_params(const CdClassifierDesc* desc, int64_t* numel);
int cd_classifier_workspace_bytes(const CdClassifierDesc* desc, int max_rows_per_call, size_t* bytes);
int cd_classifier_forward(const CdClassifierDesc* desc, const float* const* weights, const float* x, int64_t rows_total,
                          const int32_t* idx , int64_t count, float* logits, int max_rows_per_call, void* workspace,
                          size_t workspace_bytes, void* stream);
int cd_classifier_train_step(const CdClassifierDesc* desc, float* const* weights, const float* x, const float* labels, int64_t rows_total,
                             const int32_t* batch_idx, int batch, uint64_t seed, uint64_t step, float* grads, double* loss, int apply_adam,
                             float* exp_avg , float* exp_avg_sq , double lr, double beta1, double beta2, float eps,
                             int adam_step, void* workspace, size_t workspace_bytes, void* stream);
int cd_classifier_train_epoch(const CdClassifierDesc* desc, float* const* weights, const float* x, const float* labels, int64_t rows_total,
                              const int32_t* perm, int64_t n_train, int batch_size, uint64_t seed, uint64_t first_step, float* grads,
                              float* exp_avg, float* exp_avg_sq, double lr, double beta1, double beta2, float eps, double* losses,
                              void* workspace, size_t workspace_bytes, void* stream);
int cd_classifier_dropout_mask(uint64_t seed, uint64_t step, int layer, float dropout_p, int rows, int n, uint8_t* mask, void* stream);

int cd_set_conv_precision(const char* mode);
const char* cd_get_conv_precision(void);

int cd_profile_begin(void);
int cd_profile_end(char* json, int cap);

int cd_op_to_channels_last(const float* ncdhw, float* ndhwc, int batch, int channels, int64_t voxels, void* stream);
int cd_op_to_ncdhw(const float* ndhwc, float* ncdhw, int batch, int channels, int64_t voxels, void* stream);
int cd_op_cyl_conv(const float* x0, int c0, const float* x1, int c1, const float* w, const float* bias, float* y,
                   int batch, int cout, const int32_t dims_in[3], const int32_t kernel[3], const int32_t stride[3],
                   void* scratch, void* stream);
int cd_op_zslide_conv(const float* x, int cin, const float* w, const float* bias, float* y, float* ch_part, int* units, int batch,
                      int cout, const int32_t dims[3], int chunks, void* scratch, void* stream);
int cd_op_cyl_conv_transpose(const float* x, const float* w, const float* bias, float* y, int batch, int channels,
                             const int32_t dims_in[3], int kernel_z, int stride_z, const int32_t out_pad[3],
                             void* scratch, void* stream);
int cd_op_init_conv(const float* x_ncdhw, const float* w, const float* bias, float* y, int batch, int cin, int cout,
                    const int32_t dims[3], void* scratch, void* stream);
int cd_op_init_pair_conv(const float* x, const float* w0, const float* b0, const float* w1, const float* b1, int cin, const float* r_w,
                         const float* z_d, const float* phi_h, int use_rz, int use_phi, const float* scale_b, float* y, float* ch_part,
                         int* units, int batch, const int32_t dims[3], int slabs, void* scratch, void* stream);
int cd_op_group_norm(const float* x, float* y, const float* gamma, const float* beta, int batch, int channels,
                     int64_t voxels, int groups, int silu, const float* add_bc, const float* residual,
                     void* scratch, void* stream);
int cd_op_resnet_block(const float* x0, int c0, const float* x1, int c1, const float* const* w, const float* cond, float* y,
                       int batch, int cout, const int32_t dims[3], int groups, void* workspace, size_t workspace_bytes,
                       void* stream);
int cd_op_linear_attention(const float* x, const float* const* w, float* y, int batch, int channels, const int32_t dims[3],
                           void* workspace, size_t workspace_bytes, void* stream);
int cd_op_conv_backward(const float* x0, int c0, const float* x1, int c1, const float* w, const float* dy, float* dx, float* dw,
                        float* db, int batch, int cout, const int32_t dims_in[3], const int32_t kernel[3],
                        const int32_t stride[3], void* workspace, size_t workspace_bytes, void* stream);
int cd_op_conv_transpose_backward(const float* x, const float* w, const float* dy, float* dx, float* dw, float* db, int batch,
                                  int channels, const int32_t dims_in[3], int kernel_z, int stride_z, const int32_t out_pad[3],
                                  void* workspace, size_t workspace_bytes, void* stream);
int cd_op_group_norm_backward(const float* x, const float* gamma, const float* beta, const float* dy, float* dx, float* dgamma,
                              float* dbeta, float* dadd, int batch, int channels, int64_t voxels, int groups, int silu,
                              void* workspace, size_t workspace_bytes, void* stream);
size_t cd_op_scratch_bytes(int batch, int max_channels, int64_t max_voxels);
int cd_op_linear_act(const float* x, const float* w, const float* bias , float* y, int rows, int n_in, int n_out, int act,
                     float negative_slope, float dropout_p, uint64_t seed, uint64_t step, int layer, void* stream);
int cd_op_linear_act_backward(const float* x, const float* w, const float* y, const float* dy, const uint8_t* mask ,
                              float keep_scale, int act, float negative_slope, float* dx , float* dw, float* db, int rows,
                              int n_in, int n_out, void* workspace, size_t workspace_bytes, void* stream);

#ifdef __cplusplus
}
#endif
#endif
```

Before: 94.05.

## Fuse resnet block's deferred GroupNorm close into the small attention kernel

When a resnet block feeds an attention block on a small grid, the block's final GroupNorm+SiLU+residual add is left open and applied inside the attention kernel as a new pass 0. That pass also computes the PreNorm statistics in the same sweep, so no separate gn_apply launch or stats pass is needed. The cost is an extra in-place read/write of the activation inside the per-sample attention workgroup, and cooperative multi-part attention is disabled on this path. A test op entry point and an env switch to turn it off are added.

```diff
diff --git a/calodiffusion_amd/abi.py b/calodiffusion_amd/abi.py
--- a/calodiffusion_amd/abi.py
+++ b/calodiffusion_amd/abi.py
@@ -198,6 +198,8 @@
     "cd_op_resnet_block": (C.c_int, [_P, C.c_int, _P, C.c_int, C.POINTER(_P), _P, _P, C.c_int, C.c_int,
                                      C.POINTER(C.c_int32), C.c_int, _P, C.c_size_t, _P]),
     "cd_op_linear_attention": (C.c_int, [_P, C.POINTER(_P), _P, C.c_int, C.c_int, C.POINTER(C.c_int32), _P, C.c_size_t, _P]),
+    "cd_op_attn_close": (C.c_int, [_P, _P, C.c_int, _P, _P, _P, C.c_int, C.POINTER(_P), _P, C.c_int, C.c_int, C.POINTER(C.c_int32), _P,
+                                   C.c_size_t, _P]),
     "cd_op_conv_backward": (C.c_int, [_P, C.c_int, _P, C.c_int, _P, _P, _P, _P, _P, C.c_int, C.c_int, C.POINTER(C.c_int32),
                                       C.POINTER(C.c_int32), C.POINTER(C.c_int32), _P, C.c_size_t, _P]),
     "cd_op_conv_transpose_backward": (C.c_int, [_P, _P, _P, _P, _P, _P, C.c_int, C.c_int, C.POINTER(C.c_int32), C.c_int, C.c_int,
diff --git a/calodiffusion_amd/csrc/forward.hip b/calodiffusion_amd/csrc/forward.hip
--- a/calodiffusion_amd/csrc/forward.hip
+++ b/calodiffusion_amd/csrc/forward.hip
@@ -86,11 +86,6 @@
   return part;
 }
 
-struct LazyClose {
-  GnDefer gn;
-  float* part = nullptr;
-  bool on = false;
-};
 float* res_block(Run& r, const ResP& w, const float* x0, int c0, const float* x1, int c1, Dims3 dims,
                  float** part_out, int* units_out, LazyClose* lazy, float* h1_side, const ConvDone* h1_done) {
   Arena* ws = r.ws;
@@ -172,7 +167,7 @@
     if (!res) shortcut_conv();
     if (!r.dry() && !fused) launch_gn_apply(h2, h2, coef2, r.B, w.cout, vox, 1, res, nullptr, 0, po, r.s, dp2);
     ws->release(res);
-  } else if (lazy && !small && defer_gn && c1 == 0 && w.cout == 32 && !part_out) {
+  } else if (lazy && !small && defer_gn && c1 == 0 && (w.cout == 32 || lazy->attn) && !part_out) {
     lazy->gn = d2;
     lazy->part = p2;
     lazy->on = true;
@@ -186,12 +181,15 @@
   return h2;
 }
 
-float* attn_block(Run& r, const AttnP& w, const float* x, Dims3 dims, float* xpart, int xunits) {
+float* attn_block(Run& r, const AttnP& w, const float* x, Dims3 dims, float* xpart, int xunits, const LazyClose* close,
+                  const float* shortcut) {
   Arena* ws = r.ws;
   const int64_t vox = dims.vox();
   const int C = w.c;
+  CD_REQUIRE(!close || (close->on && shortcut && !xpart && attn_takes_close(vox, C)),
+             "internal: a block's close was left to an attention block that cannot take it");
   float* own = nullptr;
-  if (!xpart) {
+  if (!xpart && !close) {
     own = stats_pass(r, x, C, vox, &xunits);
     xpart = own;
   }
@@ -225,8 +223,10 @@
     yu = nsp;
     ypart = ws->get<float>((size_t)r.B * cap * C * 2);
     if (!r.dry() && single) {
+      AttnClose ac;
+      if (close) { ac.gn = close->gn; ac.shortcut = shortcut; ac.pre_gamma = w.ng; ac.pre_beta = w.nb; }
       launch_attn_small(x, C, coefn, w.qkv16, part, w.ow, kAttnScale, w.ob, w.gg, w.gb, y, ypart, r.B, vox,
-                        r.s, dnp, r.status, cap, w.coop_sync);
+                        r.s, dnp, r.status, cap, w.coop_sync, close ? &ac : nullptr);
     } else if (!r.dry()) {
       launch_attn_kv_context(x, C, coefn, w.qkv16, part, r.B, vox, nsp, r.s, dnp, r.status, momb);
       if (sep_combine) {
@@ -267,6 +267,25 @@
   }
   ws->release(ypart);
   ws->release(coefg);
+  return y;
+}
+
+float* res_then_attn(Run& r, const ResP& rw, const AttnP& aw, float* x, int cx, Dims3 dims) {
+  LazyClose lz;
+  lz.attn = !rw.has_res && cx == rw.cout && aw.c == rw.cout && attn_takes_close(dims.vox(), rw.cout);
+  float* xp = nullptr;
+  int xu = 0;
+  float* t = res_block(r, rw, x, cx, nullptr, 0, dims, lz.attn ? nullptr : &xp, &xu, lz.attn ? &lz : nullptr);
+  CD_REQUIRE(lz.on == lz.attn, "internal: the block before an attention block did not leave its close open");
+  if (!lz.on) r.ws->release(x);
+  float* y = attn_block(r, aw, t, dims, xp, xu, lz.on ? &lz : nullptr, lz.on ? x : nullptr);
+  if (lz.on) {
+    r.ws->release(lz.part);
+    r.ws->release(x);
+  } else {
+    r.ws->release(xp);
+  }
+  r.ws->release(t);
   return y;
 }
 
@@ -351,14 +370,10 @@
                          i == 0 ? first : nullptr);
     r.ws->release(x);
     x = t; cx = p->downs[i].r1.cout;
-    float* xp = nullptr;
-    int xu = 0;
-    t = res_block(r, resolve(p, p->downs[i].r2, emb), x, cx, nullptr, 0, dims, d.block_attn ? &xp : nullptr, &xu);
-    r.ws->release(x);
-    x = t;
     if (d.block_attn) {
-      t = attn_block(r, resolve(p, p->downs[i].attn), x, dims, xp, xu);
-      r.ws->release(xp);
+      x = res_then_attn(r, resolve(p, p->downs[i].r2, emb), resolve(p, p->downs[i].attn), x, cx, dims);
+    } else {
+      t = res_block(r, resolve(p, p->downs[i].r2, emb), x, cx, nullptr, 0, dims);
       r.ws->release(x);
       x = t;
     }
@@ -406,14 +421,10 @@
       r.ws->release(x);
       r.ws->release(skips[lv]);
       x = t; cx = p->ups[i].r1.cout;
-      float* up = nullptr;
-      int uu = 0;
-      t = res_block(r, resolve(p, p->ups[i].r2, emb), x, cx, nullptr, 0, dims, d.block_attn ? &up : nullptr, &uu);
-      r.ws->release(x);
-      x = t;
       if (d.block_attn) {
-        t = attn_block(r, resolve(p, p->ups[i].attn), x, dims, up, uu);
-        r.ws->release(up);
+        x = res_then_attn(r, resolve(p, p->ups[i].r2, emb), resolve(p, p->ups[i].attn), x, cx, dims);
+      } else {
+        t = res_block(r, resolve(p, p->ups[i].r2, emb), x, cx, nullptr, 0, dims);
         r.ws->release(x);
         x = t;
       }
diff --git a/calodiffusion_amd/csrc/kernels_attn.h b/calodiffusion_amd/csrc/kernels_attn.h
--- a/calodiffusion_amd/csrc/kernels_attn.h
+++ b/calodiffusion_amd/csrc/kernels_attn.h
@@ -18,11 +18,18 @@
                          hipStream_t s, float* ctx_out = nullptr, float* kstat_out = nullptr);
 
 int attn_fused_nsplit_for(int64_t vox, int batch);
+struct AttnClose {
+  GnDefer gn;
+  const float* shortcut = nullptr;
+  const float *pre_gamma = nullptr, *pre_beta = nullptr;
+};
+bool attn_takes_close(int64_t vox, int C);
 bool attn_small_eligible(int64_t vox);
 void launch_attn_small(const float* x, int C, const float* coef, const void* wqkv_f16x2, float* partials, const float* w_out,
                        float scale, const float* bias, const float* out_gamma, const float* out_beta, float* y, float* ch_part,
                        int batch, int64_t vox, hipStream_t s, const GnDefer* defer, int* status = nullptr,
-                       int max_parts = 1, unsigned* coop_sync = nullptr);
+                       int max_parts = 1, unsigned* coop_sync = nullptr,
+                       const AttnClose* close = nullptr );
 constexpr int kAttnCoopSamples = 8192;
 bool attn_moments_eligible(int C);
 size_t attn_moment_floats(int batch, int nsplit);
diff --git a/calodiffusion_amd/csrc/kernels_attn.hip b/calodiffusion_amd/csrc/kernels_attn.hip
--- a/calodiffusion_amd/csrc/kernels_attn.hip
+++ b/calodiffusion_amd/csrc/kernels_attn.hip
@@ -30,6 +30,9 @@
   unsigned* sync;
   int coop;
   float* mom;
+  GnDefer close;
+  const float* close_res;
+  const float *pre_gamma, *pre_beta;
 };
 constexpr int ATTN_MOM = 32 + 1024;
 __device__ __forceinline__ float attn_peer_load(const float* p, int coop) {
@@ -89,6 +92,16 @@
 }
 __device__ __forceinline__ void attn_barrier_lds() { asm volatile("s_waitcnt lgkmcnt(0)\n\ts_barrier" ::: "memory"); }
 template <int NCH>
+__device__ __forceinline__ void gather_coef(const float* base, int half, f32x4 (&cf)[NCH][8]) {
+#pragma unroll
+  for (int ch = 0; ch < NCH; ++ch)
+#pragma unroll
+    for (int i = 0; i < 8; ++i) {
+      const float* p = base + (ch * 32 + (i >> 2) * 16 + half * 8 + 2 * (i & 3)) * 4;
+      cf[ch][i] = f32x4{p[0], p[1], p[4], p[5]};
+    }
+}
+template <int NCH>
 __device__ __forceinline__ void load_coef(const AttnArgs& a, int b, int half, f32x4 (&cf)[NCH][8]) {
   __shared__ __attribute__((aligned(16))) float sCoef[NCH * 32 * 4];
   __shared__ __attribute__((aligned(16))) char sDefer[NCH * 32 * 16 + 64 * 8];
@@ -97,13 +110,82 @@
     gn_defer_to_lds(a.defer, b, sCoef, sDefer);
     base = sCoef;
   }
-#pragma unroll
-  for (int ch = 0; ch < NCH; ++ch)
-#pragma unroll
-    for (int i = 0; i < 8; ++i) {
-      const float* p = base + (ch * 32 + (i >> 2) * 16 + half * 8 + 2 * (i & 3)) * 4;
-      cf[ch][i] = f32x4{p[0], p[1], p[4], p[5]};
-    }
+  gather_coef<NCH>(base, half, cf);
+}
+
+template <int NCH>
+__device__ __forceinline__ void attn_close_pass0(const AttnArgs& a, int b, float* coef_lds) {
+  constexpr int C = NCH * 32, U = 8;
+  __shared__ __attribute__((aligned(16))) float sGn[C * 4];
+  __shared__ __attribute__((aligned(16))) char sDefer[C * 16 + 64 * 8];
+  __shared__ double sWave[8][2];
+  __shared__ float sStat[2];
+  const int tid = threadIdx.x;
+  gn_defer_to_lds(a.close, b, sGn, sDefer);
+  f32x4* const hb = (f32x4*)(const_cast<float*>(a.x) + (size_t)b * a.vox * C);
+  const f32x4* const rb = (const f32x4*)(a.close_res + (size_t)b * a.vox * C);
+  const int64_t n4 = a.vox * C / 4;
+  f32x4 s1 = {0.f, 0.f, 0.f, 0.f}, s2 = {0.f, 0.f, 0.f, 0.f};
+  for (int64_t i0 = tid; i0 < n4; i0 += U * 512) {
+    f32x4 t[U], r[U];
+#pragma unroll
+    for (int u = 0; u < U; ++u) {
+      const int64_t i = i0 + u * 512;
+      if (i < n4) {
+        t[u] = hb[i];
+        r[u] = rb[i];
+      }
+    }
+#pragma unroll
+    for (int u = 0; u < U; ++u) {
+      const int64_t i = i0 + u * 512;
+      if (i < n4) {
+        const int c = (int)((i * 4) % C);
+        f32x4 o;
+#pragma unroll
+        for (int e = 0; e < 4; ++e) {
+          const float2 cf = *(const float2*)(sGn + (c + e) * 4);
+          float v = cf.x * t[u][e] + cf.y;
+          v = v * __builtin_amdgcn_rcpf(1.f + __builtin_amdgcn_exp2f(v * -1.4426950408889634f));
+          o[e] = v + r[u][e];
+        }
+        hb[i] = o;
+        s1 += o;
+        s2 += o * o;
+      }
+    }
+  }
+  double a1 = ((double)s1[0] + (double)s1[1]) + ((double)s1[2] + (double)s1[3]);
+  double a2 = ((double)s2[0] + (double)s2[1]) + ((double)s2[2] + (double)s2[3]);
+#pragma unroll
+  for (int m = 32; m >= 1; m >>= 1) {
+    a1 += __shfl_xor(a1, m, 64);
+    a2 += __shfl_xor(a2, m, 64);
+  }
+  if ((tid & 63) == 0) {
+    sWave[tid >> 6][0] = a1;
+    sWave[tid >> 6][1] = a2;
+  }
+  __syncthreads();
+  if (tid == 0) {
+    double t1 = 0.0, t2 = 0.0;
+    for (int w = 0; w < 8; ++w) {
+      t1 += sWave[w][0];
+      t2 += sWave[w][1];
+    }
+    const double cnt = (double)a.vox * C;
+    const double mu = t1 / cnt;
+    double var = t2 / cnt - mu * mu;
+    var = var < 0.0 ? 0.0 : var;
+    sStat[0] = (float)mu;
+    sStat[1] = (float)(1.0 / sqrt(var + 1e-5));
+  }
+  __syncthreads();
+  if (tid < C) {
+    const float sc = sStat[1] * a.pre_gamma[tid];
+    *(f32x4*)(coef_lds + tid * 4) = f32x4{sc, a.pre_beta[tid] - sStat[0] * sc, 0.f, 0.f};
+  }
+  __syncthreads();
 }
 
 template <int NCH, bool MOM>
@@ -664,7 +746,7 @@
   attn_pass2<NCH, MOM>(a, b, unit, (int)gridDim.x, t0, t1, cf, sTr, cfl);
 }
 
-template <int NCH>
+template <int NCH, bool CLOSE>
 __global__ void __launch_bounds__(512) attn_small_kernel(AttnArgs a) {
   __shared__ __attribute__((aligned(16))) float sOut[NCH * 32][2];
   __shared__ double sTot[2];
@@ -672,7 +754,15 @@
   const int b = blockIdx.x;
   const int64_t T = (a.vox + 31) / 32;
   f32x4 cf[NCH][8];
-  load_coef<NCH>(a, b, half, cf);
+  if constexpr (CLOSE) {
+    __shared__ __attribute__((aligned(16))) float sPre[NCH * 32 * 4];
+    attn_close_pass0<NCH>(a, b, sPre);
+    gather_coef<NCH>(sPre, half, cf);
+    __threadfence_block();
+    __syncthreads();
+  } else {
+    load_coef<NCH>(a, b, half, cf);
+  }
   __shared__ __attribute__((aligned(16))) f32x4 sCfT[2 * NCH * 8];
   const f32x4* cfl = nullptr;
   if constexpr (AttnCfl<NCH, false>::value) cfl = attn_cf_table<NCH>(cf, sCfT);
@@ -905,21 +995,30 @@
   static const int max_vox = getenv("CD_ATTN_SMALL_MAX") ? atoi(getenv("CD_ATTN_SMALL_MAX")) : 1024;
   return vox <= max_vox;
 }
+static int attn_coop_parts() {
+  static const int parts = getenv("CD_ATTN_COOP") ? atoi(getenv("CD_ATTN_COOP")) : 0;
+  return parts;
+}
 void launch_attn_small(const float* x, int C, const float* coef, const void* wqkv_f16x2, float* partials, const float* w_out,
                        float scale, const float* bias, const float* out_gamma, const float* out_beta, float* y, float* ch_part,
-                       int batch, int64_t vox, hipStream_t s, const GnDefer* defer, int* status, int max_parts, unsigned* coop_sync) {
+                       int batch, int64_t vox, hipStream_t s, const GnDefer* defer, int* status, int max_parts, unsigned* coop_sync,
+                       const AttnClose* close) {
   CD_REQUIRE(C == 32 || C == 64 || C == 96 || C == 128, "fused attention: 32..128 channels");
   CD_REQUIRE((vox * C) % 4 == 0, "fused attention: whole float4 rows");
+  CD_REQUIRE(!close || (attn_takes_close(vox, C) && close->gn.part && close->gn.C == C && close->gn.groups <= 64 && close->gn.vox == vox &&
+                        close->shortcut && close->pre_gamma && close->pre_beta),
+             "fused attention: the close of the preceding block needs its partials, its shortcut and the PreNorm's parameters");
   AttnArgs a{};
   a.status = status;
   a.x = x; a.coef = coef; a.wqkv = (const u32x4*)wqkv_f16x2; a.C = C; a.vox = vox; a.tiles_per_wg = tiles_per_wg_for(vox, 1);
   a.partials = partials; a.nsplit = 1; a.wT = nullptr; a.fold_wout = w_out; a.fold_scale = scale; a.bias = bias;
   a.y = y; a.ch_part = ch_part; a.out_gamma = out_gamma; a.out_beta = out_beta;
-  if (defer) a.defer = *defer;
+  if (defer && !close) a.defer = *defer;
+  if (close) { a.close = close->gn; a.close_res = close->shortcut; a.pre_gamma = close->pre_gamma; a.pre_beta = close->pre_beta; }
   char cat[64];
   std::snprintf(cat, sizeof cat, "attn_small C%d n%ld", C, (long)vox);
-  prof::Scope scope(cat, s, 2.0 * (4.0 * C + 32) * 32 * (double)vox * batch, 4.0 * batch * (double)vox * C * 3);
-  static const int coop_env = getenv("CD_ATTN_COOP") ? atoi(getenv("CD_ATTN_COOP")) : 0;
+  prof::Scope scope(cat, s, 2.0 * (4.0 * C + 32) * 32 * (double)vox * batch, 4.0 * batch * (double)vox * C * (close ? 5 : 3));
+  const int coop_env = close ? 0 : attn_coop_parts();
   const int64_t T = (vox + 31) / 32;
   int P = coop_env < max_parts ? coop_env : max_parts;
   while (P > 1 && ((int64_t)batch * P > 256 || T < 4 * P)) --P;
@@ -942,13 +1041,29 @@
     }
   }
   const dim3 grid((unsigned)batch);
+  if (close) {
+    switch (C / 32) {
+      case 1: hipLaunchKernelGGL((attn_small_kernel<1, true>), grid, dim3(512), 0, s, a); break;
+      case 2: hipLaunchKernelGGL((attn_small_kernel<2, true>), grid, dim3(512), 0, s, a); break;
+      case 3: hipLaunchKernelGGL((attn_small_kernel<3, true>), grid, dim3(512), 0, s, a); break;
+      default: hipLaunchKernelGGL((attn_small_kernel<4, true>), grid, dim3(512), 0, s, a); break;
+    }
+    CD_HIP(hipGetLastError());
+    return;
+  }
   switch (C / 32) {
-    case 1: hipLaunchKernelGGL(attn_small_kernel<1>, grid, dim3(512), 0, s, a); break;
-    case 2: hipLaunchKernelGGL(attn_small_kernel<2>, grid, dim3(512), 0, s, a); break;
-    case 3: hipLaunchKernelGGL(attn_small_kernel<3>, grid, dim3(512), 0, s, a); break;
-    default: hipLaunchKernelGGL(attn_small_kernel<4>, grid, dim3(512), 0, s, a); break;
+    case 1: hipLaunchKernelGGL((attn_small_kernel<1, false>), grid, dim3(512), 0, s, a); break;
+    case 2: hipLaunchKernelGGL((attn_small_kernel<2, false>), grid, dim3(512), 0, s, a); break;
+    case 3: hipLaunchKernelGGL((attn_small_kernel<3, false>), grid, dim3(512), 0, s, a); break;
+    default: hipLaunchKernelGGL((attn_small_kernel<4, false>), grid, dim3(512), 0, s, a); break;
   }
   CD_HIP(hipGetLastError());
 }
 
-}
+bool attn_takes_close(int64_t vox, int C) {
+  static const bool fused_env = getenv("CD_NO_FUSED_ATTN") == nullptr && getenv("CD_NO_GNDEFER") == nullptr;
+  return fused_env && conv_precision() == PREC_F16X2 && vox > 128 && attn_small_eligible(vox) && attn_coop_parts() <= 1 &&
+         (C == 32 || C == 64 || C == 96 || C == 128) && getenv("CD_NO_ATTN_CLOSE") == nullptr;
+}
+
+}
diff --git a/calodiffusion_amd/csrc/ops.hip b/calodiffusion_amd/csrc/ops.hip
--- a/calodiffusion_amd/csrc/ops.hip
+++ b/calodiffusion_amd/csrc/ops.hip
@@ -1,4 +1,7 @@
 #include "plan_internal.h"
+#include "kernels_attn.h"
+
+#include <cstdlib>
 
 namespace cd {
 
@@ -237,6 +240,47 @@
   });
 }
 
+int cd_op_attn_close(const float* c2, const float* ch_part, int units, const float* shortcut, const float* gamma, const float* beta,
+                     int groups, const float* const* w, float* y, int batch, int channels, const int32_t dims[3], void* workspace,
+                     size_t workspace_bytes, void* stream) {
+  return guarded([&] {
+    CD_REQUIRE(c2 && ch_part && units > 0 && shortcut && gamma && beta && w && y && workspace, "bad argument");
+    CD_REQUIRE(groups > 0 && groups <= 64 && channels % groups == 0, "group norm: <= 64 groups dividing the channels");
+    hipStream_t s = (hipStream_t)stream;
+    Arena ws;
+    ws.reset((char*)workspace, workspace_bytes, false);
+    float* pq = ws.get<float>(packed_weight_floats(channels, 96, 1));
+    launch_pack_weights(w[2], pq, 96, channels, 1, false, s);
+    float* pq16 = ws.get<float>(packed_f16x2_bytes(channels, 96, 1) / 4);
+    launch_pack_weights_f16x2(w[2], pq16, 96, channels, 1, s);
+    AttnP a;
+    a.c = channels; a.ng = w[0]; a.nb = w[1]; a.qkv = pq; a.ow = w[3]; a.ob = w[4]; a.gg = w[5]; a.gb = w[6];
+    a.qkv16 = pq16;
+    Run run{&ws, s, batch, groups};
+    const Dims3 d{dims[0], dims[1], dims[2]};
+    const int64_t vox = d.vox();
+    float* h = ws.get<float>((size_t)batch * vox * channels);
+    CD_HIP(hipMemcpyAsync(h, c2, sizeof(float) * (size_t)batch * vox * channels, hipMemcpyDeviceToDevice, s));
+    LazyClose lz;
+    lz.gn.part = ch_part; lz.gn.units = units; lz.gn.gamma = gamma; lz.gn.beta = beta; lz.gn.C = channels; lz.gn.groups = groups;
+    lz.gn.vox = vox;
+    float* out = nullptr;
+    if (attn_takes_close(vox, channels)) {
+      lz.on = lz.attn = true;
+      out = attn_block(run, a, h, d, nullptr, 0, &lz, shortcut);
+    } else {
+      const int bps = gn_apply_blocks_per_sample(batch, channels, vox);
+      float* po = ws.get<float>((size_t)batch * bps * channels * 2);
+      float* coef = ws.get<float>((size_t)batch * channels * 4);
+      const bool defer = getenv("CD_NO_GNDEFER") == nullptr;
+      if (!defer) launch_gn_finalize(ch_part, units, gamma, beta, nullptr, 0, coef, batch, channels, groups, vox, s);
+      launch_gn_apply(h, h, coef, batch, channels, vox, 1, shortcut, nullptr, 0, po, s, defer ? &lz.gn : nullptr);
+      out = attn_block(run, a, h, d, po, bps);
+    }
+    CD_HIP(hipMemcpyAsync(y, out, sizeof(float) * (size_t)batch * vox * channels, hipMemcpyDeviceToDevice, s));
+  });
+}
+
 int cd_op_conv_backward(const float* x0, int c0, const float* x1, int c1, const float* w, const float* dy, float* dx, float* dw,
                         float* db, int batch, int cout, const int32_t dims_in[3], const int32_t kernel[3],
                         const int32_t stride[3], void* workspace, size_t workspace_bytes, void* stream) {
diff --git a/calodiffusion_amd/csrc/plan_internal.h b/calodiffusion_amd/csrc/plan_internal.h
--- a/calodiffusion_amd/csrc/plan_internal.h
+++ b/calodiffusion_amd/csrc/plan_internal.h
@@ -233,7 +233,12 @@
   const HeadArgs* upd = nullptr;
 };
 
-struct LazyClose;
+struct LazyClose {
+  GnDefer gn;
+  float* part = nullptr;
+  bool on = false;
+  bool attn = false;
+};
 float* stats_pass(Run& r, const float* x, int C, int64_t vox, int* units);
 float* conv3_with_stats(Run& r, const float* x0, int c0, const float* x1, int c1, const float* wpk, const void* wpk3,
                         const float* bias, float* out, int cout, Dims3 dims, const float* coef_in, int* units,
@@ -246,7 +251,9 @@
 float* res_block(Run& r, const ResP& w, const float* x0, int c0, const float* x1, int c1, Dims3 dims,
                  float** part_out = nullptr, int* units_out = nullptr, LazyClose* lazy = nullptr, float* h1_side = nullptr,
                  const ConvDone* h1_done = nullptr);
-float* attn_block(Run& r, const AttnP& w, const float* x, Dims3 dims, float* xpart = nullptr, int xunits = 0);
+float* attn_block(Run& r, const AttnP& w, const float* x, Dims3 dims, float* xpart = nullptr, int xunits = 0,
+                  const LazyClose* close = nullptr, const float* shortcut = nullptr);
+float* res_then_attn(Run& r, const ResP& rw, const AttnP& aw, float* x, int cx, Dims3 dims);
 void bias_grad(Run& r, const float* dy, int C, int64_t vox, float* db);
 void conv_backward(Run& r, const float* x0, int c0, const float* x1, int c1, const float* w_raw, const float* dy, float* dx,
                    float* dw, float* db, int cout, const ConvGeom& g, const DgImg* img = nullptr, const float* xcoef = nullptr,
diff --git a/calodiffusion_amd/engine.py b/calodiffusion_amd/engine.py
--- a/calodiffusion_amd/engine.py
+++ b/calodiffusion_amd/engine.py
@@ -234,7 +234,7 @@
         self._weights_version = ver
 
     _WS_SWITCHES = ("CD_NO_DEEP_LEVEL", "CD_NO_PW_CLOSE", "CD_NO_FUSED_ATTN", "CD_NO_GNDEFER", "CD_ATTN_COMBINE_LAUNCH", "CD_PW_F32",
-                    "CD_NO_ATTN_MOMENTS", "CD_ATTN_MOM_MIN", "CD_NO_DEEP_SIDE_CONV")
+                    "CD_NO_ATTN_MOMENTS", "CD_ATTN_MOM_MIN", "CD_NO_DEEP_SIDE_CONV", "CD_NO_ATTN_CLOSE")
 
     def _ws_key(self, batch: int):
         return (int(batch),) + tuple(os.environ.get(k) for k in self._WS_SWITCHES)
diff --git a/calodiffusion_amd/ops.py b/calodiffusion_amd/ops.py
--- a/calodiffusion_amd/ops.py
+++ b/calodiffusion_amd/ops.py
@@ -183,3 +183,15 @@
         _check(self.lib.cd_op_linear_attention(x.data_ptr(), ptrs, y.data_ptr(), B, c, _i32x3((D, H, W)), ws.data_ptr(),
                                                ws.numel(), _stream()))
         return y
+
+    def attn_close(self, c2_cl, part, shortcut_cl, gamma, beta, sd: Dict[str, torch.Tensor], groups=8):
+        c2, sc, part = _dev32(c2_cl, "c2"), _dev32(shortcut_cl, "shortcut"), _dev32(part, "part")
+        B, D, H, W, c = c2.shape
+        assert sc.shape == c2.shape and part.shape[0] == B and tuple(part.shape[2:]) == (c, 2)
+        ptrs = (_P * 7)(*[sd[k].data_ptr() for k in self._ATTN_KEYS])
+        y = torch.empty_like(c2)
+        nbytes = self.lib.cd_op_scratch_bytes(B, 96, D * H * W) + 4 * B * D * H * W * 96 * 4
+        ws = torch.empty(nbytes, dtype=torch.uint8, device=c2.device)
+        _check(self.lib.cd_op_attn_close(c2.data_ptr(), part.data_ptr(), part.shape[1], sc.data_ptr(), gamma.data_ptr(), beta.data_ptr(),
+                                         groups, ptrs, y.data_ptr(), B, c, _i32x3((D, H, W)), ws.data_ptr(), ws.numel(), _stream()))
+        return y
diff --git a/include/calodiff.h b/include/calodiff.h
--- a/include/calodiff.h
+++ b/include/calodiff.h
@@ -339,6 +339,9 @@
                        void* stream);
 int cd_op_linear_attention(const float* x, const float* const* w, float* y, int batch, int channels, const int32_t dims[3],
                            void* workspace, size_t workspace_bytes, void* stream);
+int cd_op_attn_close(const float* c2, const float* ch_part, int units, const float* shortcut, const float* gamma, const float* beta,
+                     int groups, const float* const* w, float* y, int batch, int channels, const int32_t dims[3], void* workspace,
+                     size_t workspace_bytes, void* stream);
 int cd_op_conv_backward(const float* x0, int c0, const float* x1, int c1, const float* w, const float* dy, float* dx, float* dw,
                         float* db, int batch, int cout, const int32_t dims_in[3], const int32_t kernel[3],
                         const int32_t stride[3], void* workspace, size_t workspace_bytes, void* stream);
```

After: 94.67, median of 6. About the same (+0.7%).
